# ChangwuLiu/InGVIO

Hardware: AMD Instinct MI355X
Metric: ekf_updates_per_sec (higher is better)
Workload: dtype f64; 1 GPU; BASELINE configs[1]: synthetic stereo MSCKF, 150 feats x 11 clones, state dim N=249 (update at N), 512 independent filters per GPU; step = propagate(k=10)+clone+MSCKF update+marginalise; filters_per_gpu=512, feats=150, clones=11, state_dim=249, imu_steps=10, parallelism=independent filters, 1 rank(s), no data-path collective

## Files before the change

### ingvio_amd/csrc/capi.hip

```cpp
#include "../../include/ingvio_hip.h"
#include "dev_common.h"
#include "launch_ekf.h"
#include "launch_msckf.h"
#include "launch_factored.h"
#include "launch_tri.h"
#include "launch_tracks.h"
#include "launch_lm.h"
#include "launch_delayed.h"
#include "launch_qr.h"
#include "launch_chol.h"
#include "launch_gnss.h"
#include "launch_lmbatch.h"
#include "launch_nominal.h"
#include "launch_tail.h"

#include <stdio.h>
#include <stdlib.h>
#include <string.h>
#include <unistd.h>
#include <string>
#include <atomic>
#include <cmath>
#include <condition_variable>
#include <functional>
#include <mutex>
#include <thread>
#include <utility>
#include <vector>

#define KMAX 64
#ifndef UPLOAD_KERNEL_MAX
#define UPLOAD_KERNEL_MAX (256u << 10)
#endif
#define IMU_SLAB_NB 4
#define CHI2_CAP 1024

namespace {

enum ProfId { PF_RESTORE, PF_PROPAGATE, PF_AUGMENT, PF_GATE, PF_FOLD, PF_MERGE, PF_EKF_CORE, PF_DOWNDATE, PF_MARG,
              PF_GATE2, PF_GRAM, PF_INFO, PF_APPLY, PF_ROWGATE, PF_LM_BUILD, PF_LM_GEMM, PF_LM_CHOL, PF_POSTCOLS, PF_COUNT };
const char* kProfNames[PF_COUNT] = { "restore", "k_propagate", "k_augment", "k_msckf_gate", "k_msckf_fold",
                                     "k_msckf_merge", "k_ekf_core", "k_downdate", "k_marginalize",
                                     "gate", "gram", "solve", "apply", "k_rows_gate",
                                     "k_lm_build", "k_lm_gemm", "k_lm_chol", "k_post_cols" };
struct ProfRec { int id; hipEvent_t a, b; };

}

struct ingvio_ctx {
    ingvio_ctx_desc d;
    int ldp, mld, nc_cap, G, rstride, hstride, cstride, ystride;
    int cls;
    hipStream_t st;
    bool own_stream;
    std::string err;
    double *Pbase, *Psnap;
    size_t pp = 0;
    int *d_cur, *d_n, *d_n_snap;
    std::vector<int> h_n, h_cur, h_n_snap;
    bool has_snap;
    int prof_only = -1;
    bool strip_ok = false;
    std::vector<int> h_nclones;
    struct { double *e = nullptr, *o = nullptr, *r = nullptr, *f = nullptr; int cap = 0; } se;
    bool phase_restore = false;
    unsigned long long mut_seq = 0, strip_seq = 0;
    double *d_Phi, *d_G, *d_dt, *d_R, *d_blk;
    double* d_prm = nullptr;
    int *d_gnss, *d_idx;
    int* d_zero_idx = nullptr;
    char* d_result_slab = nullptr;
    char* h_result = nullptr;
    size_t result_bytes = 0, ro_gam = 0, ro_used = 0, ro_m = 0, ro_st = 0, ro_tok = 0, ro_tpf = 0;
    char* d_frame_slab[2] = { nullptr, nullptr };
    int *d_clone_idx, *d_nclones, *d_nfeat, *d_anchor, *d_dof;
    double *d_clone_R, *d_clone_p, *d_pf, *d_uv, *d_chi2;
    unsigned long long* d_mask;
    double *d_gamma, *d_Rpart, *d_H, *d_res, *d_noise, *d_noise1, *d_Y, *d_Yc, *d_dx, *d_rec, *d_hnew;
    int method;
    int *d_accept, *d_used, *d_chunk_used, *d_colmap, *d_m, *d_nc, *d_status, *d_pcbase;
    double *d_big_sg, *d_big_wk;
    double* d_Asum = nullptr;
    int* d_used_sum = nullptr;
    struct { std::vector<double> chi2; bool chi2_ok = false; double var = 0.0; int b0 = -1, nb = 0; bool noise_ok = false; } upc;
    int apply_flipped = 0;
    bool fork_recorded = false;
    unsigned long long* d_tri_mask = nullptr;
    char* d_imu = nullptr;
    double* d_Tflat = nullptr;

    int* d_tri_ok;
    struct QrCache { int m = 0, n = 0, ldh = 0, chol = 0; double *dA = nullptr, *db = nullptr, *ws = nullptr, *dT = nullptr; hipGraphExec_t exec = nullptr; } qr;
    int qr_method = 0;
    double* d_noiseB = nullptr;
    struct GnssStage {
        double *H = nullptr, *res = nullptr, *noise = nullptr, *gamma = nullptr, *chi2 = nullptr;
        int *m = nullptr, *nc = nullptr, *colmap = nullptr, *keep = nullptr;
        double *feph = nullptr, *fobs = nullptr, *frcv = nullptr, *front = nullptr;
        int ncw = 0, m_cap = 0, n_vars_hi = 0, chi2_len = 0, gate_rows = 0, strong = 0;
        double thr1 = 0.0;
        std::vector<int> hi;
        bool staged = false;
        bool in_frame = false, fused_last = false;
        bool folded_last = false;
        bool results = false;
        int nc_max = 0;
        double *W = nullptr, *Yf = nullptr, *dxf = nullptr;
        int *mf = nullptr, *ncf = nullptr;
        bool nominal = false, nom_pending = false, own_status = false;
        bool frame_nom = false;
        int nom_b0 = 0, nom_nb = 0;
        int* stf = nullptr;
    } gn;
    struct DenseWs {
        double *Hd = nullptr, *X = nullptr, *Y = nullptr, *Tb = nullptr, *U = nullptr, *noise = nullptr, *noiseB = nullptr;
        int *m = nullptr, *cidx = nullptr, *rowmap = nullptr;
        int m_cap = 0, n_ld = 0, n32 = 0, ldx = 0;
        size_t hstride = 0, xstride = 0, tstride = 0, ustride = 0;
    } dw;
    struct LmStage {
        double *pose = nullptr, *pf = nullptr, *uv = nullptr, *gamma = nullptr, *dx = nullptr;
        int *idx = nullptr, *n_lm = nullptr, *lm_idx = nullptr, *anchor_idx = nullptr, *tracked = nullptr, *accept = nullptr;
        LmOpts op;
        int l_hi = 0, in_frame = 0;
        bool alloc = false, staged = false;
        int* slot = nullptr;
        bool nominal = false, nom_pending = false;
        int nom_b0 = 0, nom_nb = 0;
        std::vector<int> hi;
    } lm;
    char* d_multi = nullptr;
    struct DelayedWs { char *in = nullptr, *wk = nullptr, *out = nullptr, *h_out = nullptr; size_t in_cap = 0, wk_cap = 0, out_cap = 0; } dl;
    size_t multi_cap = 0;
    int st_stereo, st_enable_gnss, st_fmax_used;
    std::vector<double> st_prm;
    MsckfOpts st_op;
    std::vector<int> st_gnss;
    std::vector<int> st_marg;
    std::vector<int> st_cidx_hi;
    bool staged;
    double* d_xchg = nullptr;
    bool phase_pending = false;
    struct InputSet {
        double *Phi = nullptr, *G = nullptr, *dt = nullptr, *R = nullptr, *clone_R = nullptr, *clone_p = nullptr, *pf = nullptr, *uv = nullptr,
               *chi2 = nullptr, *noise = nullptr, *prm = nullptr;
        int *gnss = nullptr, *idx = nullptr, *clone_idx = nullptr, *nclones = nullptr, *nfeat = nullptr, *anchor = nullptr, *dof = nullptr;
        unsigned long long* mask = nullptr;
    } alt;
    bool alt_ready = false;
    hipStream_t st2 = nullptr;
    hipEvent_t ev_fork = nullptr, ev_join = nullptr, ev_ref = nullptr;
    hipEvent_t ev_fetch = nullptr;
    int fetch_b0 = 0, fetch_nb = 0;
    hipStream_t st_copy = nullptr;
    hipEvent_t ev_copy = nullptr, ev_free[2] = { nullptr, nullptr };
    bool copy_pending = false, free_valid[2] = { false, false };
    int set_id = 0;
    struct PinSlab { char* p = nullptr; size_t cap = 0; hipEvent_t ev = nullptr; bool busy = false; };
    PinSlab pin[4];
    int pin_next = 0;
    struct PartStream { hipStream_t st = nullptr; hipEvent_t ev_gate = nullptr, ev_apply = nullptr, ev_done = nullptr; };
    PartStream part[4];
    int parts_alloc = 0;
    int parts_req = -1;
    bool split_pending = false;
    hipEvent_t tok_last = nullptr;
    hipEvent_t ev_split_fork = nullptr;
    hipStream_t run_st = nullptr;
    hipEvent_t tok_wait = nullptr, tok_rec = nullptr;
    struct Tracks { double *uv = nullptr, *pf = nullptr; unsigned long long* mask = nullptr; int t_max = 0; char* stage[2] = { nullptr, nullptr }; size_t stage_cap = 0; } trk;
    struct Nominal {
        int vmax = 0, ir = 0, dr = 0;
        int* ih = nullptr; double* dv = nullptr;
        int* ih_snap = nullptr; double* dv_snap = nullptr;
        double* dx = nullptr;
        std::vector<int> h_ih, h_ih_snap;
        bool has_snap = false;
        bool pending = false;
        bool frame = false;
        hipEvent_t ev = nullptr; bool ev_valid = false;
    } nom;
    struct TailWs { char *in = nullptr, *ws = nullptr, *h_out = nullptr; size_t in_cap = 0, ws_cap = 0, out_cap = 0; } tl;
    bool prof;
    std::vector<ProfRec> recs;
    double prof_ms[PF_COUNT];
    int prof_calls[PF_COUNT];
};

namespace {

#define HIPCHK(ctx, expr)                                                                       \
    do {                                                                                        \
        hipError_t e__ = (expr);                                                                \
        if (e__ != hipSuccess) {                                                                \
            (ctx)->err = std::string(#expr) + ": " + hipGetErrorString(e__);                    \
            return INGVIO_E_HIP;                                                                \
        }                                                                                       \
    } while (0)

template <class T>
int dalloc(ingvio_ctx* c, T** p, size_t count)
{
    HIPCHK(c, hipMalloc((void**)p, sizeof(T) * (count ? count : 1)));
    HIPCHK(c, hipMemsetAsync(*p, 0, sizeof(T) * (count ? count : 1), c->st));
    return 0;
}

CovView view(ingvio_ctx* c)
{
    CovView v;
    v.Pbase = c->Pbase; v.cur = c->d_cur; v.n = c->d_n; v.ldp = c->ldp; v.B = c->d.batch; v.pstride = c->pp;
    ++c->mut_seq;
    return v;
}

FrameView fview(ingvio_ctx* c)
{
    FrameView f;
    f.clone_idx = c->d_clone_idx; f.clone_R = c->d_clone_R; f.clone_p = c->d_clone_p;
    f.n_clones = c->d_nclones; f.n_feat = c->d_nfeat; f.pf = c->d_pf; f.anchor = c->d_anchor;
    f.obs_mask = c->d_mask; f.uv = c->d_uv; f.dof = c->d_dof; f.cmax = c->d.c_max; f.fmax = c->d.f_max;
    return f;
}

struct ProfScope {
    ingvio_ctx* c; int id; hipEvent_t a, b; bool on;
    ProfScope(ingvio_ctx* c_, int id_) : c(c_), id(id_), on(c_->prof && (c_->prof_only < 0 || c_->prof_only == id_))
    {
        if (on) { hipEventCreate(&a); hipEventCreate(&b); hipEventRecord(a, c->run_st); }
    }
    ~ProfScope()
    {
        if (on) { hipEventRecord(b, c->run_st); c->recs.push_back({ id, a, b }); }
    }
};

int check_range(ingvio_ctx* c, int b0, int nb)
// ... 359 lines not shown
           pad64(8 * n * fm * cm * 4) + pad64(8 * n * fm) + 1024;
}

int validate_frames(ingvio_ctx* c, int b0, int nb, const ingvio_msckf_frame* fr, int grow, int* fmax_used)
{
    const int cm = c->d.c_max, fm = c->d.f_max;
    int fmx = 0;
    for (int i = 0; i < nb; ++i) {
        const ingvio_msckf_frame& f = fr[i];
        if (f.n_clones < 0 || f.n_clones > cm || f.n_feat < 0 || f.n_feat > fm) return INGVIO_E_CAPACITY;
        if (f.n_clones > 0 && (!f.clone_idx || !f.clone_R || !f.clone_p)) return INGVIO_E_ARG;
        if (f.n_feat > 0 && (!f.obs_mask || !f.uv)) return INGVIO_E_ARG;
        if (f.n_feat > fmx) fmx = f.n_feat;
        const int n_live = grow >= 0 ? c->h_n[b0 + i] + grow : c->d.n_max;
        const int n_lim = n_live < c->d.n_max ? n_live : c->d.n_max;
        for (int s = 0; s < f.n_clones; ++s) {
            if (f.clone_idx[s] < 0) return INGVIO_E_ARG;
            if (f.clone_idx[s] + 6 > n_lim) return f.clone_idx[s] + 6 > c->d.n_max ? INGVIO_E_ARG : INGVIO_E_NOT_IN_STATE;
        }
        if (f.anchor)
            for (int j = 0; j < f.n_feat; ++j) if (f.anchor[j] < 0 || f.anchor[j] >= f.n_clones) return INGVIO_E_ARG;
    }
    if (fmax_used) *fmax_used = fmx;
    return 0;
}

int pack_frames(ingvio_ctx* c, Uploader& up, int b0, int nb, const ingvio_msckf_frame* fr, int* fmax_used)
{
    const int cm = c->d.c_max, fm = c->d.f_max;
    int fmx = 0;
    for (int i = 0; i < nb; ++i) if (fr[i].n_feat > fmx) fmx = fr[i].n_feat;
    const bool whole = b0 == 0 && nb == c->d.batch;
    up.off = (up.off + 63) & ~(size_t)63;
    const size_t slab0 = up.off;
    int* cidx = up.take<int>((size_t)nb * cm); int* ncl = up.take<int>(nb); int* nft = up.take<int>(nb);
    int* anc = up.take<int>((size_t)nb * fm); int* dof = up.take<int>((size_t)nb * fm);
    double* cR = up.take<double>((size_t)nb * cm * 9); double* cp = up.take<double>((size_t)nb * cm * 3);
    double* pf = up.take<double>((size_t)nb * fm * 3);
    unsigned long long* mk = up.take<unsigned long long>((size_t)nb * fm);
    double* uv = up.take<double>((size_t)nb * fm * cm * 4);
    parallel_for(nb, [=](int i) {
        const ingvio_msckf_frame& f = fr[i];
        const int C = f.n_clones, F = f.n_feat;
        ncl[i] = C; nft[i] = F;
        memcpy(cidx + (size_t)i * cm, f.clone_idx, sizeof(int) * (size_t)C);
        memcpy(cR + (size_t)i * cm * 9, f.clone_R, 72 * (size_t)C);
        memcpy(cp + (size_t)i * cm * 3, f.clone_p, 24 * (size_t)C);
        if (f.pf) memcpy(pf + (size_t)i * fm * 3, f.pf, 24 * (size_t)F); else memset(pf + (size_t)i * fm * 3, 0, 24 * (size_t)F);
        if (f.anchor) memcpy(anc + (size_t)i * fm, f.anchor, sizeof(int) * (size_t)F); else memset(anc + (size_t)i * fm, 0, sizeof(int) * (size_t)F);
        if (f.dof) memcpy(dof + (size_t)i * fm, f.dof, sizeof(int) * (size_t)F); else memset(dof + (size_t)i * fm, 0, sizeof(int) * (size_t)F);
        const unsigned long long cmask = C >= 64 ? ~0ULL : ((1ULL << C) - 1ULL);
        unsigned long long* mki = mk + (size_t)i * fm;
        for (int j = 0; j < F; ++j) mki[j] = f.obs_mask[j] & cmask;
        for (int j = F; j < fm; ++j) mki[j] = 0ULL;
        double* uvi = uv + (size_t)i * fm * cm * 4;
        if (C == cm) memcpy(uvi, f.uv, 32 * (size_t)F * C);
        else for (int j = 0; j < F; ++j) memcpy(uvi + (size_t)j * cm * 4, f.uv + (size_t)j * C * 4, 32 * (size_t)C);
    });
    for (int i = 0; i < nb; ++i) c->h_nclones[b0 + i] = fr[i].n_clones;
    if (whole) {
        const size_t used = (size_t)(reinterpret_cast<char*>(uv) - (up.slab->p + slab0)) + 8 * ((size_t)(nb - 1) * fm + (size_t)fr[nb - 1].n_feat) * cm * 4;
        up.copy(reinterpret_cast<char*>(c->d_clone_idx), up.slab->p + slab0, std::max(used, (size_t)64));
        *fmax_used = fmx;
        return 0;
    }
    up.copy(c->d_clone_idx + (size_t)b0 * cm, cidx, (size_t)nb * cm);
    up.copy(c->d_nclones + b0, ncl, nb);
    up.copy(c->d_nfeat + b0, nft, nb);
    up.copy(c->d_anchor + (size_t)b0 * fm, anc, (size_t)nb * fm);
    up.copy(c->d_dof + (size_t)b0 * fm, dof, (size_t)nb * fm);
    up.copy(c->d_clone_R + (size_t)b0 * cm * 9, cR, (size_t)nb * cm * 9);
    up.copy(c->d_clone_p + (size_t)b0 * cm * 3, cp, (size_t)nb * cm * 3);
    up.copy(c->d_pf + (size_t)b0 * fm * 3, pf, (size_t)nb * fm * 3);
    up.copy(c->d_uv + (size_t)b0 * fm * cm * 4, uv, (size_t)nb * fm * cm * 4);
    up.copy(c->d_mask + (size_t)b0 * fm, mk, (size_t)nb * fm);
    *fmax_used = fmx;
    return 0;
}

int stage_frames(ingvio_ctx* c, int b0, int nb, const ingvio_msckf_frame* fr, int* fmax_used, int grow = 0)
{
    int rc = validate_frames(c, b0, nb, fr, grow, nullptr);
    if (rc) return rc;
    if (wait_inputs(c)) return INGVIO_E_HIP;
    Uploader up{ c };
    rc = up.begin(frames_bytes(c, nb));
    if (rc) return rc;
    pack_frames(c, up, b0, nb, fr, fmax_used);
    return up.end();
}

void fill_opts(const ingvio_ctx* c, const ingvio_msckf_opts* o, MsckfOpts* op)
{
    memcpy(op->R_lr, o->R_cl2cr, 72);
    memcpy(op->t_lr, o->t_cl2cr, 24);
    op->var = o->noise * o->noise;
    op->max_accept = o->max_accept;
    op->selected_variant = o->selected_variant;
    op->chi2 = c->d_chi2;
    op->chi2_len = o->chi2_len;
}

int make_opts(ingvio_ctx* c, const ingvio_msckf_opts* o, MsckfOpts* op)
{
    if (!o || !o->chi2_table || o->chi2_len < 2 || o->chi2_len > CHI2_CAP) return INGVIO_E_ARG;
    fill_opts(c, o, op);
    if (wait_inputs(c)) return INGVIO_E_HIP;
    auto& u = c->upc;
    if (u.chi2_ok && (int)u.chi2.size() >= o->chi2_len && !memcmp(u.chi2.data(), o->chi2_table, 8 * (size_t)o->chi2_len)) return 0;
    const UpItem item = { c->d_chi2, o->chi2_table, 8 * (size_t)o->chi2_len };
    if (stage_small(c, &item, 1)) return INGVIO_E_HIP;
    u.chi2.assign(o->chi2_table, o->chi2_table + o->chi2_len); u.chi2_ok = true;
    return 0;
}

#define GNSS_NCW 32

void gnss_front_launch(ingvio_ctx* c, int b0, int nb, bool nominal, hipStream_t st);
static int gnss_in_frame_launch(ingvio_ctx* c, int b0, int nb, FactoredLaunch& L)
{
    auto& g = c->gn;
    const size_t mld = c->mld, hs = mld * GNSS_NCW, ws = (size_t)c->ldp * 16;
    L.gcolmap = g.colmap + (size_t)b0 * GNSS_NCW; L.gnc = g.nc + b0; L.gcstride = GNSS_NCW;
    L.gW = g.W + (size_t)b0 * ws; L.gWstride = ws;
    if (g.frame_nom) {
        L.stage = 10; launch_factored(L, c->run_st);
        launch_nominal_update(nom_table(c), c->d_dx, c->ldp, nullptr, b0, nb, c->run_st);
        gnss_front_launch(c, b0, nb, true, c->run_st);
    }
    { ProfScope p(c, PF_POSTCOLS); L.stage = 4; launch_factored(L, c->run_st); }
    EkfLaunch E;
    memset(&E, 0, sizeof E);
    E.cv = L.cv; E.b0 = b0; E.nb = nb; E.H = c->d_H + (size_t)b0 * hs; E.res = c->d_res + (size_t)b0 * mld;
    E.colmap = c->d_colmap + (size_t)b0 * GNSS_NCW; E.m = g.mf + b0; E.nc = g.ncf + b0;
    E.noise = c->d_noiseB + (size_t)b0 * mld; E.r_kind = INGVIO_R_DIAG; E.mld = c->mld; E.hstride = (int)hs; E.cstride = GNSS_NCW;
    E.nstride = c->mld; E.Y = g.Yf + (size_t)b0 * ws; E.ystride = (int)ws; E.dx = g.dxf;
    E.status = g.own_status ? g.stf : c->d_status; E.m_cap = g.m_cap; E.nc_cap = GNSS_NCW;
    E.W = L.gW; E.wstride = ws; E.ypad = 16; E.marg_idx = L.marg_idx; E.marg_size = L.marg_size;
    if (g.strong) { E.chi2 = g.chi2; E.chi2_len = g.chi2_len; E.gate_max_rows = 14; }
    RowsGateIn in{ g.H + (size_t)b0 * hs, g.res + (size_t)b0 * mld, g.noise + (size_t)b0 * mld, g.m + b0, g.colmap + (size_t)b0 * GNSS_NCW,
                   g.nc + b0, (int)hs, GNSS_NCW };
    {
        ProfScope p(c, PF_ROWGATE);
        if (launch_rows_gate(E, in, g.thr1, g.gamma + (size_t)b0 * mld, g.keep + (size_t)b0 * mld, c->run_st)) return INGVIO_E_CAPACITY;
    }
    { ProfScope p(c, PF_EKF_CORE); launch_ekf_core(E, c->run_st); }
    L.gY = E.Y; L.gYstride = ws; L.gm = g.mf + b0;
    g.fused_last = true; g.folded_last = true;
    g.results = true;
    return 0;
}

int run_msckf_factored(ingvio_ctx* c, int b0, int nb, const MsckfOpts& op, int stereo, int fmax_used,
                       const int* marg_idx = nullptr, int marg_size = 0, int phase = 0, bool gnss_fuse = false)
{
    FactoredLaunch L;
    memset(&L, 0, sizeof L);
    L.stereo = stereo; L.cv = view(c); L.fv = fview(c); L.op = op; L.b0 = b0; L.nb = nb;
    L.fmax_used = fmax_used > 0 ? fmax_used : 1;
    L.ncol_cap = 6 * c->d.c_max;
    for (int i = 0; i < nb; ++i) if (c->h_nclones[b0 + i] > L.c_used) L.c_used = c->h_nclones[b0 + i];
    L.gamma = c->d_gamma; L.accept = c->d_accept; L.used = c->d_used; L.rec = c->d_rec;
    L.Apart = c->d_Rpart + (size_t)b0 * c->G * c->rstride; L.chunk_used = c->d_chunk_used + (size_t)b0 * c->G;
    L.G = c->G; L.rstride = c->rstride; L.noise = c->d_noise + b0;
    L.Tflat = c->d_Tflat; L.tfstride = (size_t)c->ldp * 100; L.flat_nb = std::min(c->d.batch, APPLY_FLAT_NB);
    L.Asum = c->d_Asum ? c->d_Asum + (size_t)b0 * c->rstride : nullptr; L.used_sum = c->d_used_sum ? c->d_used_sum + b0 : nullptr;
#ifdef INGVIO_ALT_KERNELS
    static const bool few_off = [] { const char* e = getenv("INGVIO_FEW"); return e && !strcmp(e, "off"); }();
    if (few_off) { L.Tflat = nullptr; L.Asum = nullptr; }
#endif
    L.T = c->d_Y + (size_t)b0 * c->ystride; L.Pc = c->d_Yc + (size_t)b0 * c->ystride; L.ystride = c->ystride;
    L.dx = c->d_dx; L.m_out = c->d_m + b0; L.nc_out = c->d_nc + b0; L.status = c->d_status;
    L.big_sg = c->d_big_sg ? c->d_big_sg + (size_t)b0 * bigwin_sg_doubles(c->G) : nullptr;
    L.big_wk = c->d_big_wk ? c->d_big_wk + (size_t)b0 * bigwin_wk_doubles() : nullptr;
    const bool big = c->d.c_max > 16;
    L.mstride = c->ystride; L.n_cap = c->d.n_max;
    L.marg_idx = marg_idx; L.marg_size = marg_size; L.pc_base = c->d_pcbase + b0;
    c->apply_flipped = 0;
    L.flip_cnt = c->d_pcbase + c->d.batch + b0; L.did_flip = no_apply_flip() ? nullptr : &c->apply_flipped;
    bool forked = false;
    if (big && phase == 0 && c->st2) {
        if (!c->fork_recorded) HIPCHK(c, hipEventRecord(c->ev_fork, c->run_st));
        c->fork_recorded = false;
        forked = true;
    }
    if (phase != 2) {
        if (c->tok_wait) HIPCHK(c, hipStreamWaitEvent(c->run_st, c->tok_wait, 0));
        {
            const bool pon = c->prof && (c->prof_only < 0 || c->prof_only == PF_GATE2);
            int used = 0;
            if (pon) { hipEventCreate(&L.prof_a); hipEventCreate(&L.prof_b); L.prof_used = &used; }
            L.stage = 0;
            const int grc = launch_factored(L, c->run_st);
            if (pon) {
                if (used) c->recs.push_back({ PF_GATE2, L.prof_a, L.prof_b });
                else { hipEventDestroy(L.prof_a); hipEventDestroy(L.prof_b); }
                L.prof_a = nullptr; L.prof_b = nullptr; L.prof_used = nullptr;
            }
            if (grc) return INGVIO_E_UNSUPPORTED;
        }
        { ProfScope p(c, PF_GRAM); L.stage = 1; launch_factored(L, c->run_st); }
        if (c->tok_rec) HIPCHK(c, hipEventRecord(c->tok_rec, c->run_st));
    }
    if (forked) {
        HIPCHK(c, hipStreamWaitEvent(c->st2, c->ev_fork, 0));
        L.stage = 6; launch_factored(L, c->st2);
        HIPCHK(c, hipEventRecord(c->ev_ref, c->st2));
        L.stage = 7; launch_factored(L, c->st2);
        HIPCHK(c, hipEventRecord(c->ev_join, c->st2));
    }
    if (phase == 1) return last_launch(c);
    if (forked) {
        ProfScope p(c, PF_INFO);
        HIPCHK(c, hipStreamWaitEvent(c->run_st, c->ev_ref, 0));
        L.stage = 8; launch_factored(L, c->run_st);
        HIPCHK(c, hipStreamWaitEvent(c->run_st, c->ev_join, 0));
        L.stage = 9; launch_factored(L, c->run_st);
    } else {
        if (big) { ProfScope p(c, PF_INFO); L.stage = 5; launch_factored(L, c->run_st); }
        { ProfScope p(c, PF_INFO); L.stage = 2; launch_factored(L, c->run_st); }
    }
    if (gnss_fuse) { if (int rc = gnss_in_frame_launch(c, b0, nb, L)) return rc; }
    if (phase == 2 && c->tok_wait) HIPCHK(c, hipStreamWaitEvent(c->run_st, c->tok_wait, 0));
    { ProfScope p(c, PF_APPLY); L.stage = 3; launch_factored(L, c->run_st); }
    if (phase == 2 && c->tok_rec) HIPCHK(c, hipEventRecord(c->tok_rec, c->run_st));
    return last_launch(c);
}

int run_msckf(ingvio_ctx* c, int b0, int nb, const MsckfOpts& op, int stereo, int fmax_used)
{
    if (c->method == 1) return run_msckf_factored(c, b0, nb, op, stereo, fmax_used);
    MsckfLaunch L;
    memset(&L, 0, sizeof L);
    L.stereo = stereo; L.cv = view(c); L.fv = fview(c); L.op = op; L.b0 = b0; L.nb = nb;
    L.fmax_used = fmax_used > 0 ? fmax_used : 1;
    L.gamma = c->d_gamma; L.accept = c->d_accept; L.used = c->d_used;
    L.Rpart = c->d_Rpart + (size_t)b0 * c->G * c->rstride; L.chunk_used = c->d_chunk_used + (size_t)b0 * c->G;
    L.G = c->G; L.rstride = c->rstride;
    L.Hout = c->d_H + (size_t)b0 * c->hstride; L.res_out = c->d_res + (size_t)b0 * c->mld;
    L.colmap = c->d_colmap + (size_t)b0 * c->cstride; L.m_out = c->d_m + b0; L.nc_out = c->d_nc + b0;
    L.mld = c->mld; L.hstride = c->hstride; L.cstride = c->cstride;
    { ProfScope p(c, PF_GATE); L.stage = 0; if (launch_msckf(L, c->st)) return INGVIO_E_UNSUPPORTED; }
    { ProfScope p(c, PF_FOLD); L.stage = 1; launch_msckf(L, c->st); }
    { ProfScope p(c, PF_MERGE); L.stage = 2; launch_msckf(L, c->st); }
    EkfLaunch E;
    memset(&E, 0, sizeof E);
    E.cv = view(c); E.b0 = b0; E.nb = nb; E.H = L.Hout; E.res = L.res_out; E.colmap = L.colmap; E.m = L.m_out; E.nc = L.nc_out;
    E.noise = c->d_noise + b0; E.r_kind = 0; E.mld = c->mld; E.hstride = c->hstride; E.cstride = c->cstride; E.nstride = 1;
    E.Y = c->d_Y + (size_t)b0 * c->ystride; E.ystride = c->ystride; E.dx = c->d_dx; E.status = c->d_status;
    E.m_cap = 6 * c->d.c_max; E.nc_cap = 6 * c->d.c_max;
    { ProfScope p(c, PF_EKF_CORE); launch_ekf_core(E, c->st); }
    { ProfScope p(c, PF_DOWNDATE); launch_downdate(E, c->d.n_max, c->st); }
    return last_launch(c);
}

int fill_noise_scalar(ingvio_ctx* c, int b0, int nb, double var)
{
    auto& u = c->upc;
    if (u.noise_ok && u.b0 == b0 && u.nb == nb && u.var == var) return 0;
    std::vector<double> v(nb, var);
    const UpItem item = { c->d_noise + b0, v.data(), 8 * (size_t)nb };
    if (stage_small(c, &item, 1)) return INGVIO_E_HIP;
    u.noise_ok = true; u.b0 = b0; u.nb = nb; u.var = var;
    return 0;
}

template <class Step>
int stage_imu_params(ingvio_ctx* c, int b0, int nb, const Step* steps, const double sigma[4], double scb, double srw, double* blk, int* count)
{
    const bool all = !c->staged;
    const int lo = all ? 0 : b0, hi = all ? c->d.batch : b0 + nb;
    for (int b = lo; b < hi; ++b) {
        double* h = &c->st_prm[(size_t)b * 8];
        h[0] = sigma[0]; h[1] = sigma[1]; h[2] = sigma[2]; h[3] = sigma[3]; h[4] = scb; h[5] = srw;
        h[6] = (double)steps[b >= b0 && b < b0 + nb ? b - b0 : 0].k; h[7] = 0.0;
        memcpy(blk + (size_t)(b - lo) * 8, h, 64);
    }
    *count = hi - lo;
    return lo;
}

struct FrameStage {
    ingvio_ctx* c; int b0, nb; const ingvio_msckf_opts* opts; const double* sigma; int enable_gnss; double scb, srw; bool async;
    Uploader upl{ c };
    int refuse(bool inputs, bool tracks) const
    {
        if (phase_busy(c)) return INGVIO_E_ARG;
        if (c && c->nom.pending) { c->err = "a frame staged from the device nominal state has not run yet"; return INGVIO_E_ARG; }
        if (check_range(c, b0, nb) || !inputs || !opts || !sigma) return INGVIO_E_ARG;
        if (tracks && !c->trk.t_max) { c->err = "ingvio_frame_stage_tracks without ingvio_tracks_create"; return INGVIO_E_ARG; }
        if (async && (b0 != 0 || nb != c->d.batch)) return INGVIO_E_ARG;
        if (!opts->chi2_table || opts->chi2_len < 2 || opts->chi2_len > CHI2_CAP) return INGVIO_E_ARG;
        return 0;
    }
    int begin(size_t bytes)
    {
        if (async) if (int rc = prepare_async_set(c)) return rc;
        return upl.begin(bytes + pad64(8 * CHI2_CAP) + pad64(8 * (size_t)nb) + pad64(64 * (size_t)c->d.batch) + 1024);
    }
    int fail(int code)
    {
        hipStreamSynchronize(c->st);
        if (c->st_copy) hipStreamSynchronize(c->st_copy);
        c->staged = false; c->copy_pending = false;
        return code;
    }
    template <class Step>
    int commit(const Step* steps)
    {
        bool same = c->staged && enable_gnss == c->st_enable_gnss;
        for (int i = 0; i < nb; ++i)
            for (int g = 0; g < 5; ++g) {
                int& old = c->st_gnss[(size_t)(b0 + i) * 5 + g];
                if (old != steps[i].gnss_idx[g]) { same = false; old = steps[i].gnss_idx[g]; }
            }
// ... 2817 lines not shown
    return INGVIO_OK;
}

static bool lm_in_frame(const ingvio_ctx* c) { return c->lm.staged && c->lm.in_frame; }
static bool gnss_in_frame(const ingvio_ctx* c) { return c->gn.staged && c->gn.in_frame && c->gn.m_cap > 0; }
static bool gnss_folds(const ingvio_ctx* c)
{
    if (!gnss_in_frame(c) || c->d.c_max > 16 || c->gn.m_cap > 16 || c->gn.nc_max > 16) return false;
    for (int b = 0; b < c->d.batch; ++b) if (c->st_marg[b] < 0 || c->gn.hi[b] > c->st_marg[b]) return false;
    return true;
}

static bool strips_valid(const ingvio_ctx* c, int restore_prior) { return restore_prior && c->strip_ok && c->mut_seq == c->strip_seq; }

static void launch_restore_propagate(ingvio_ctx* c, int restore_prior, bool strips, int b0, int nb, hipStream_t st)
{
    const bool from_snap = strips && propagate_can_restore(c->d.n_max) && !no_snap_propagate();
    if (restore_prior && !from_snap) {
        ProfScope p(c, PF_RESTORE);
        if (strips) launch_restore_strips(view(c), b0, nb, c->d.n_max, c->Psnap, c->d_n_snap, c->st_enable_gnss ? c->d_gnss : nullptr, st);
        else launch_restore(view(c), b0, nb, c->d.n_max, c->Psnap, c->d_n_snap, st);
    }
    ProfScope p(c, PF_PROPAGATE);
    const ImuLaunch im = imu_launch(c, b0, nb);
    launch_propagate(view(c), b0, nb, c->d.n_max, c->d_Phi + (size_t)b0 * KMAX * 225, c->d_G + (size_t)b0 * KMAX * 180, c->d_dt + (size_t)b0 * KMAX,
                     im.k, KMAX, im.prm, c->st_enable_gnss ? c->d_gnss + (size_t)b0 * 5 : nullptr, im.sigma, c->st_enable_gnss, im.scb, im.srw, st,
                     c->d_R + (size_t)b0 * 9, c->d_status, from_snap ? c->Psnap : nullptr, c->d_n_snap);
}

static void mirror_restore_clone(ingvio_ctx* c, int restore_prior)
{
    if (restore_prior) { c->h_n = c->h_n_snap; std::fill(c->h_cur.begin(), c->h_cur.end(), 0); }
    for (int b = 0; b < c->d.batch; ++b) c->h_n[b] += 6;
}
static bool mirror_marg(ingvio_ctx* c)
{
    bool all = true;
    for (int b = 0; b < c->d.batch; ++b) { if (c->st_marg[b] >= 0) { c->h_n[b] -= 6; c->h_cur[b] ^= 1; } else all = false; }
    return all;
}

static void consume_in_frame(bool& staged, bool in_frame, bool replay) { if (staged && in_frame && !replay) staged = false; }
static void strips_after_step(ingvio_ctx* c, bool valid) { c->strip_ok = valid; c->strip_seq = c->mut_seq; }

static int frame_run_split(ingvio_ctx* c, int restore_prior, int P, bool gnss_fuse)
{
    const int B = c->d.batch;
    if (parts_prepare(c, P)) return INGVIO_E_HIP;
    if (c->split_pending && c->copy_pending) ENTER(c);
    if (wait_inputs(c)) return INGVIO_E_HIP;
    if (!c->split_pending) {
        HIPCHK(c, hipEventRecord(c->ev_split_fork, c->st));
        for (int p = 0; p < P; ++p) HIPCHK(c, hipStreamWaitEvent(c->part[p].st, c->ev_split_fork, 0));
        c->tok_last = nullptr;
    }
    const bool strips = strips_valid(c, restore_prior);
    mirror_restore_clone(c, restore_prior);
    int rc = 0;
    auto range = [&](int p, int& b0, int& nb) {
        b0 = (int)((long long)B * p / P) & ~7;
        const int b1 = p + 1 == P ? B : ((int)((long long)B * (p + 1) / P) & ~7);
        nb = b1 - b0;
    };
    for (int p = 0; p < P && !rc; ++p) {
        int b0, nb; range(p, b0, nb);
        if (nb <= 0) continue;
        auto& q = c->part[p];
        c->run_st = q.st;
        launch_restore_propagate(c, restore_prior, strips, b0, nb, q.st);
        c->tok_wait = c->tok_last; c->tok_rec = q.ev_gate;
        rc = run_msckf_factored(c, b0, nb, c->st_op, c->st_stereo, c->st_fmax_used, c->d_idx + b0, 6, 1, gnss_fuse);
        c->tok_last = rc ? nullptr : q.ev_gate;
    }
    for (int p = 0; p < P && !rc; ++p) {
        int b0, nb; range(p, b0, nb);
        if (nb <= 0) continue;
        auto& q = c->part[p];
        c->run_st = q.st;
        c->tok_wait = c->tok_last; c->tok_rec = q.ev_apply;
        rc = run_msckf_factored(c, b0, nb, c->st_op, c->st_stereo, c->st_fmax_used, c->d_idx + b0, 6, 2, gnss_fuse);
        c->tok_last = rc ? nullptr : q.ev_apply;
        if (!rc && !c->apply_flipped) {
            ProfScope pr(c, PF_MARG);
            launch_post_marg(view(c), b0, nb, c->d_idx + b0, 6, q.st);
        }
    }
    for (int p = 0; p < P; ++p) hipEventRecord(c->part[p].ev_done, c->part[p].st);
    c->tok_wait = nullptr; c->tok_rec = nullptr;
    c->run_st = c->st;
    c->split_pending = true;
    if (rc) { c->tok_last = nullptr; ENTER(c); return rc; }
    const bool all_marg = mirror_marg(c);
    strips_after_step(c, all_marg && restore_prior);
    consume_in_frame(c->gn.staged, c->gn.in_frame, restore_prior != 0);
    return INGVIO_OK;
}

static int frame_run_front(ingvio_ctx* c, int restore_prior)
{
    const int B = c->d.batch;
    ENTER(c);
    if (wait_inputs(c)) return INGVIO_E_HIP;
    launch_restore_propagate(c, restore_prior, strips_valid(c, restore_prior), 0, B, c->st);
    mirror_restore_clone(c, restore_prior);
    strips_after_step(c, false);
    const int rc = run_msckf_factored(c, 0, B, c->st_op, c->st_stereo, c->st_fmax_used, nullptr, 0, 1);
    if (rc == 0) { c->phase_pending = true; c->phase_restore = restore_prior != 0; }
    return rc;
}

static int frame_run_back(ingvio_ctx* c)
{
    c->phase_pending = false;
    const int B = c->d.batch;
    const bool with_lm = lm_in_frame(c), replay = c->phase_restore;
    int rc = run_msckf_factored(c, 0, B, c->st_op, c->st_stereo, c->st_fmax_used, with_lm ? nullptr : c->d_idx, with_lm ? 0 : 6, 2);
    if (rc) return rc;
    if (with_lm) { rc = landmark_update_launch(c, 0, B); if (rc) return rc; }
    {
        ProfScope p(c, PF_MARG);
        if (!with_lm) { if (!c->apply_flipped) launch_post_marg(view(c), 0, B, c->d_idx, 6, c->st); }
        else launch_marginalize(view(c), 0, B, c->d.n_max, c->d_idx, 6, c->st);
    }
    mirror_marg(c);
    consume_in_frame(c->lm.staged, c->lm.in_frame, replay);
    strips_after_step(c, false);
    if (gnss_in_frame(c)) {
        rc = gnss_run_separate(c, 0, B, true);
        if (rc) return rc;
        consume_in_frame(c->gn.staged, c->gn.in_frame, replay);
    }
    return release_input_set(c);
}

static int frame_run_whole(ingvio_ctx* c, int restore_prior)
{
    const int B = c->d.batch;
    ENTER(c);
    if (wait_inputs(c)) return INGVIO_E_HIP;
    launch_restore_propagate(c, restore_prior, strips_valid(c, restore_prior), 0, B, c->st);
    mirror_restore_clone(c, restore_prior);
    const bool with_lm = lm_in_frame(c);
    const bool fuse = c->method == 1 && !with_lm;
    const bool lm_oop = with_lm && c->method == 1;
    const bool gnss_here = gnss_in_frame(c), gnss_fuse = fuse && gnss_folds(c);
    const bool gnss_nomf = c->gn.staged && c->gn.frame_nom;
    if (gnss_nomf) {
        auto& g = c->gn;
        HIPCHK(c, hipMemsetAsync(g.dxf, 0, 8 * (size_t)B * c->ldp, c->st));
        HIPCHK(c, hipMemsetAsync(g.stf, 0, sizeof(int) * (size_t)B, c->st));
        HIPCHK(c, hipMemsetAsync(g.mf, 0, sizeof(int) * (size_t)B, c->st));
        g.own_status = true; g.results = true; g.fused_last = true; g.folded_last = false;
    }
    int rc = fuse     ? run_msckf_factored(c, 0, B, c->st_op, c->st_stereo, c->st_fmax_used, c->d_idx, 6, 0, gnss_fuse)
             : lm_oop ? run_msckf_factored(c, 0, B, c->st_op, c->st_stereo, c->st_fmax_used, c->d_zero_idx, 0)
                      : run_msckf(c, 0, B, c->st_op, c->st_stereo, c->st_fmax_used);
    if (rc) return rc;
    if (lm_oop) {
        if (!c->apply_flipped) launch_post_marg(view(c), 0, B, c->d_zero_idx, 0, c->st);
        for (int b = 0; b < B; ++b) c->h_cur[b] ^= 1;
    }
    const bool lm_nom = with_lm && c->lm.nominal;
    if (lm_nom) landmark_gather_launch(c, c->d_dx, 0, B);
    bool lm_fused = false;
    if (with_lm) { rc = landmark_update_launch(c, 0, B, c->d_idx, 6, &lm_fused); if (rc) return rc; }
    if (!(fuse && c->apply_flipped)) {
        ProfScope p(c, PF_MARG);
        if (fuse || lm_fused) launch_post_marg(view(c), 0, B, c->d_idx, 6, c->st);
        else launch_marginalize(view(c), 0, B, c->d.n_max, c->d_idx, 6, c->st);
    }
    consume_in_frame(c->lm.staged, c->lm.in_frame, restore_prior != 0);
    const bool all_marg = mirror_marg(c);
    if (c->nom.pending) {
        if (gnss_nomf && gnss_fuse) launch_nominal_update_post(nom_table(c), c->gn.dxf, c->ldp, c->d_idx, 0, B, c->st);
        else launch_nominal_update(nom_table(c), lm_nom ? c->lm.dx : c->d_dx, c->ldp, c->d_idx, 0, B, c->st);
        if (int rc2 = last_launch(c)) return rc2;
        for (int b = 0; b < B; ++b) nom_mirror_marg(c, b, c->st_marg[b]);
        c->nom.pending = false;
        if (nom_mark(c)) return INGVIO_E_HIP;
    }
    strips_after_step(c, fuse && all_marg && restore_prior);
    if (gnss_here && !gnss_fuse) {
        if (gnss_nomf) {
            for (int b = 0; b < B; ++b) { int& hi = c->gn.hi[b]; if (c->st_marg[b] >= 0 && hi > c->st_marg[b]) hi -= 6; }
            gnss_front_launch(c, 0, B, true, c->st);
        }
        rc = gnss_run_separate(c, 0, B, true);
        if (rc) return rc;
        if (gnss_nomf) {
            launch_nominal_update(nom_table(c), c->gn.dxf, c->ldp, nullptr, 0, B, c->st);
            if (int rc2 = last_launch(c)) return rc2;
            if (nom_mark(c)) return INGVIO_E_HIP;
        }
    }
    consume_in_frame(c->gn.staged, c->gn.in_frame, restore_prior != 0);
    if (!c->gn.staged) c->gn.frame_nom = false;
    return release_input_set(c);
}

static int frame_run_impl(ingvio_ctx* c, int restore_prior, int phase)
{
    if (!c || !c->staged) return INGVIO_E_ARG;
    if (c->nom.frame) {
        if (!c->nom.pending) { c->err = "the frame staged from the device nominal state has already run"; return INGVIO_E_ARG; }
        if (phase) { c->err = "the split step does not take a frame staged from the device nominal state"; return INGVIO_E_UNSUPPORTED; }
        if (restore_prior) { c->err = "restore_prior with a frame staged from the device nominal state (restore with ingvio_cov_restore before the stage)"; return INGVIO_E_ARG; }
        if ((c->gn.staged && c->gn.in_frame && !c->gn.frame_nom) || (lm_in_frame(c) && !c->lm.nominal) || c->parts_req > 1) {
            c->err = "the device nominal state takes no in-frame GNSS / host-fed landmark stage and frame_parts = 1 only"; return INGVIO_E_UNSUPPORTED;
        }
    } else if (lm_in_frame(c) && c->lm.nominal) {
        c->err = "an in-frame landmark stage from the device nominal state needs a frame staged from it"; return INGVIO_E_ARG;
    } else if (c->gn.staged && c->gn.frame_nom) {
        c->err = "a GNSS epoch staged for a frame from the device nominal state needs that frame"; return INGVIO_E_ARG;
    }
    if (phase && c->method != 1) return INGVIO_E_UNSUPPORTED;
    if (phase != 2 && phase_busy(c)) return INGVIO_E_ARG;
    if (phase == 2 && !c->phase_pending) { c->err = "ingvio_frame_run_phase(.., 2) without a preceding phase 1"; return INGVIO_E_ARG; }
    if (phase != 0 && c->st_op.max_accept > 0) { c->err = "max_accept is not supported by the split (feature-sharded) frame step"; return INGVIO_E_ARG; }
    if (phase == 2) return frame_run_back(c);
    const int B = c->d.batch;
    if (restore_prior && !c->has_snap) return INGVIO_E_ARG;
    if (c->method == 0 && c->d.c_max > 16) return INGVIO_E_UNSUPPORTED;
    {
        const std::vector<int>& n0 = restore_prior ? c->h_n_snap : c->h_n;
        for (int b = 0; b < B; ++b) {
            if (n0[b] < 21) return INGVIO_E_ARG;
            if (n0[b] + 6 > c->d.n_max) return INGVIO_E_CAPACITY;
            if (c->st_cidx_hi[b] + 6 > n0[b] + 6) return INGVIO_E_NOT_IN_STATE;
            if (c->st_marg[b] >= 0 && c->st_marg[b] + 6 > n0[b] + 6) return INGVIO_E_NOT_IN_STATE;
        }
        if (lm_in_frame(c)) { if (int rc = landmark_in_state(c, 0, B, n0, 6)) return rc; }
    }
    if (phase == 1) return frame_run_front(c, restore_prior);
    const int P = std::min(c->parts_req > 0 ? c->parts_req : 1, 4);
    const bool gnss_fuse = gnss_folds(c);
    if (P > 1 && c->method == 1 && !lm_in_frame(c) && c->d.c_max <= 16 && (!gnss_in_frame(c) || gnss_fuse) && B >= 16 * P)
        return frame_run_split(c, restore_prior, P, gnss_fuse);
    return frame_run_whole(c, restore_prior);
}

int ingvio_frame_run(ingvio_ctx* c, int restore_prior) { return frame_run_impl(c, restore_prior, 0); }
int ingvio_set_frame_parts(ingvio_ctx* c, int parts)
{
    if (!c || parts < -1 || parts > 4) return INGVIO_E_ARG;
    ENTER(c);
    c->parts_req = parts == 0 ? 1 : parts;
    return INGVIO_OK;
}
int ingvio_frame_run_phase(ingvio_ctx* c, int restore_prior, int phase)
{
    if (phase < 0 || phase > 2) return INGVIO_E_ARG;
    return frame_run_impl(c, restore_prior, phase);
}

int ingvio_info_set(ingvio_ctx* c, int b, const double* A, int ncol, int n_accepted)
{
    ENTER(c);
    if (check_range(c, b, 1) || !A || ncol < 6 || (size_t)ncol * (ncol + 1) > (size_t)c->rstride || n_accepted < 0) return INGVIO_E_ARG;
    std::vector<int> used(c->G, 0);
    used[0] = n_accepted;
    int rc = up(c, c->d_Rpart + (size_t)b * c->G * c->rstride, A, 8 * (size_t)ncol * (ncol + 1));
    rc |= up(c, c->d_chunk_used + (size_t)b * c->G, used.data(), sizeof(int) * (size_t)c->G);
    if (rc) return INGVIO_E_HIP;
    HIPCHK(c, hipStreamSynchronize(c->st));
    return INGVIO_OK;
}

namespace {
__global__ __launch_bounds__(256) void k_info_reduce(const double* __restrict__ Apart, const int* __restrict__ chunk_used, int G, int rstride,
                                                     int cnt, double* __restrict__ out)
{
    const int e = blockIdx.x * 256 + threadIdx.x;
    if (e > cnt) return;
    double s = 0.0;
    if (e < cnt) { for (int g = 0; g < G; ++g) if (chunk_used[g]) s += Apart[(size_t)g * rstride + e]; }
    else { for (int g = 0; g < G; ++g) s += (double)chunk_used[g]; }
    out[e] = s;
}
__global__ __launch_bounds__(256) void k_info_commit(const double* __restrict__ in, int cnt, double* __restrict__ Apart0, int* __restrict__ chunk_used, int G)
{
    const int e = blockIdx.x * 256 + threadIdx.x;
    if (e < cnt) Apart0[e] = in[e];
    if (e < G) chunk_used[e] = e == 0 ? (int)llrint(in[cnt]) : 0;
}
}

int ingvio_info_reduce(ingvio_ctx* c, int b, double** dev_ptr, int* count, int* ncol_out)
{
    ENTER(c);
    if (check_range(c, b, 1) || !dev_ptr || !count || c->method != 1) return INGVIO_E_ARG;
    int C = 0;
    if (down_sync(c, &C, c->d_nclones + b, sizeof(int))) return INGVIO_E_HIP;
    const int ncol = 6 * C, cnt = ncol * (ncol + 1);
    if (cnt <= 0 || cnt > c->rstride) return INGVIO_E_ARG;
    if (!c->d_xchg && dalloc(c, &c->d_xchg, (size_t)c->d.batch * (c->rstride + 8))) return INGVIO_E_HIP;
    double* out = c->d_xchg + (size_t)b * (c->rstride + 8);
    hipLaunchKernelGGL(k_info_reduce, dim3((cnt + 256) / 256), dim3(256), 0, c->st, c->d_Rpart + (size_t)b * c->G * c->rstride,
                       c->d_chunk_used + (size_t)b * c->G, c->G, c->rstride, cnt, out);
    HIPCHK(c, hipStreamSynchronize(c->st));
    *dev_ptr = out; *count = cnt + 1;
    if (ncol_out) *ncol_out = ncol;
    return last_launch(c);
}

int ingvio_info_commit(ingvio_ctx* c, int b)
{
    ENTER(c);
    if (check_range(c, b, 1) || !c->d_xchg || c->method != 1) return INGVIO_E_ARG;
    int C = 0;
    if (down_sync(c, &C, c->d_nclones + b, sizeof(int))) return INGVIO_E_HIP;
    const int ncol = 6 * C, cnt = ncol * (ncol + 1);
    if (cnt <= 0 || cnt > c->rstride) return INGVIO_E_ARG;
    hipLaunchKernelGGL(k_info_commit, dim3((std::max(cnt, c->G) + 255) / 256), dim3(256), 0, c->st, c->d_xchg + (size_t)b * (c->rstride + 8), cnt,
                       c->d_Rpart + (size_t)b * c->G * c->rstride, c->d_chunk_used + (size_t)b * c->G, c->G);
    return last_launch(c);
}

int ingvio_frame_fetch_begin(ingvio_ctx* c, int b0, int nb)
{
    ENTER(c);
    if (check_range(c, b0, nb)) return INGVIO_E_ARG;
    const int fm = c->d.f_max;
    if (!c->ev_fetch) HIPCHK(c, hipEventCreateWithFlags(&c->ev_fetch, hipEventDisableTiming));
    HIPCHK(c, hipMemcpyAsync(c->h_result + 8 * (size_t)b0 * c->ldp, c->d_dx + (size_t)b0 * c->ldp, 8 * (size_t)nb * c->ldp, hipMemcpyDeviceToHost, c->st));
    HIPCHK(c, hipMemcpyAsync(c->h_result + c->ro_used + sizeof(int) * (size_t)b0 * fm, c->d_used + (size_t)b0 * fm, sizeof(int) * (size_t)nb * fm, hipMemcpyDeviceToHost, c->st));
    HIPCHK(c, hipMemcpyAsync(c->h_result + c->ro_m + sizeof(int) * (size_t)b0, c->d_m + b0, sizeof(int) * (size_t)nb, hipMemcpyDeviceToHost, c->st));
    HIPCHK(c, hipEventRecord(c->ev_fetch, c->st));
    c->fetch_b0 = b0; c->fetch_nb = nb;
    return last_launch(c);
}

int ingvio_frame_fetch_end(ingvio_ctx* c, double* dx_out, int* accepted, int* rows_out)
{
    if (!c || c->fetch_nb <= 0) return INGVIO_E_ARG;
    const int fm = c->d.f_max, b0 = c->fetch_b0, nb = c->fetch_nb;
    HIPCHK(c, hipEventSynchronize(c->ev_fetch));
    c->fetch_nb = 0;
    if (dx_out) memcpy(dx_out, c->h_result + 8 * (size_t)b0 * c->ldp, 8 * (size_t)nb * c->ldp);
    if (accepted) memcpy(accepted, c->h_result + c->ro_used + sizeof(int) * (size_t)b0 * fm, sizeof(int) * (size_t)nb * fm);
    if (rows_out) memcpy(rows_out, c->h_result + c->ro_m + sizeof(int) * (size_t)b0, sizeof(int) * (size_t)nb);
    return INGVIO_OK;
}

int ingvio_frame_fetch(ingvio_ctx* c, int b0, int nb, double* dx_out, int* accepted, int* rows_out)
{
    int rc = ingvio_frame_fetch_begin(c, b0, nb);
    if (rc) return rc;
    rc = ingvio_frame_fetch_end(c, dx_out, accepted, rows_out);
    if (rc) return rc;
    HIPCHK(c, hipStreamSynchronize(c->st));
    return last_launch(c);
}

int ingvio_set_msckf_method(ingvio_ctx* c, int method)
{
    ENTER(c);
    if (!c || method < 0 || method > 1) return INGVIO_E_ARG;
    c->method = method;
    return INGVIO_OK;
}

int ingvio_debug_msckf_info(ingvio_ctx* c, int b, double* A_out, int* ncol_out)
{
    ENTER(c);
    if (check_range(c, b, 1) || !A_out || !ncol_out) return INGVIO_E_ARG;
    int C = 0;
    if (down_sync(c, &C, c->d_nclones + b, sizeof(int))) return INGVIO_E_HIP;
    const int ncol = 6 * C;
    *ncol_out = ncol;
    const size_t w = (size_t)ncol + 1;
    for (size_t e = 0; e < (size_t)ncol * w; ++e) A_out[e] = 0.0;
    if (c->method == 1) {
        std::vector<int> used(c->G);
        if (down_sync(c, used.data(), c->d_chunk_used + (size_t)b * c->G, sizeof(int) * (size_t)c->G)) return INGVIO_E_HIP;
        std::vector<double> part((size_t)ncol * w);
        for (int g = 0; g < c->G; ++g) {
            if (!used[g]) continue;
            if (down_sync(c, part.data(), c->d_Rpart + ((size_t)b * c->G + g) * c->rstride, 8 * part.size())) return INGVIO_E_HIP;
            for (size_t e = 0; e < part.size(); ++e) A_out[e] += part[e];
        }
        return INGVIO_OK;
    }
    int m = 0;
    if (down_sync(c, &m, c->d_m + b, sizeof(int))) return INGVIO_E_HIP;
    if (m == 0) return INGVIO_OK;
    std::vector<double> R((size_t)c->mld * ncol), z(c->mld);
    if (down_sync(c, R.data(), c->d_H + (size_t)b * c->hstride, 8 * R.size()) || down_sync(c, z.data(), c->d_res + (size_t)b * c->mld, 8 * (size_t)ncol))
        return INGVIO_E_HIP;
    for (int i = 0; i < ncol; ++i) {
        for (int j = 0; j < ncol; ++j) {
            double a = 0.0;
            for (int k = 0; k <= (i < j ? i : j); ++k) a += R[k + (size_t)i * c->mld] * R[k + (size_t)j * c->mld];
            A_out[i * w + j] = a;
        }
        double bb = 0.0;
        for (int k = 0; k <= i; ++k) bb += R[k + (size_t)i * c->mld] * z[k];
        A_out[i * w + ncol] = bb;
    }
    return INGVIO_OK;
}

int ingvio_debug_info_solution(ingvio_ctx* c, int b, double* out, int count)
{
    ENTER(c);
    if (check_range(c, b, 1) || !out || count < 1 || count > c->ystride) return INGVIO_E_ARG;
    if (down_sync(c, out, c->d_Y + (size_t)b * c->ystride, 8 * (size_t)count)) return INGVIO_E_HIP;
    return INGVIO_OK;
}

static int debug_quiesce(ingvio_ctx* c)
{
    HIPCHK(c, hipStreamSynchronize(c->st));
    if (c->st_copy) HIPCHK(c, hipStreamSynchronize(c->st_copy));
    return 0;
}
static int debug_down(ingvio_ctx* c, void* dst, const void* src, size_t bytes)
{
    if (dst && bytes) HIPCHK(c, hipMemcpy(dst, src, bytes, hipMemcpyDeviceToHost));
    return 0;
}

int ingvio_debug_tracks_read(ingvio_ctx* c, int b, unsigned long long* mask, double* uv, double* pf)
{
    ENTER(c);
    if (check_range(c, b, 1)) return INGVIO_E_ARG;
    if (!c->trk.t_max) { c->err = "ingvio_debug_tracks_read without ingvio_tracks_create"; return INGVIO_E_ARG; }
    if (debug_quiesce(c)) return INGVIO_E_HIP;
    const size_t T = c->trk.t_max, C = c->d.c_max;
    if (debug_down(c, mask, c->trk.mask + (size_t)b * T, 8 * T) || debug_down(c, uv, c->trk.uv + (size_t)b * T * C * 4, 8 * T * C * 4) ||
        debug_down(c, pf, c->trk.pf + (size_t)b * T * 3, 8 * T * 3)) return INGVIO_E_HIP;
    return INGVIO_OK;
}

int ingvio_debug_staged_frame(ingvio_ctx* c, int b, int* n_clones, int* n_feat, int* clone_idx, double* clone_R, double* clone_p, int* anchor, int* dof,
                              unsigned long long* obs_mask, double* pf, double* uv)
{
    ENTER(c);
    if (check_range(c, b, 1)) return INGVIO_E_ARG;
    if (debug_quiesce(c)) return INGVIO_E_HIP;
    const size_t cm = c->d.c_max, fm = c->d.f_max, B = b;
    if (debug_down(c, n_clones, c->d_nclones + B, 4) || debug_down(c, n_feat, c->d_nfeat + B, 4) ||
        debug_down(c, clone_idx, c->d_clone_idx + B * cm, 4 * cm) || debug_down(c, clone_R, c->d_clone_R + B * cm * 9, 8 * cm * 9) ||
        debug_down(c, clone_p, c->d_clone_p + B * cm * 3, 8 * cm * 3) || debug_down(c, anchor, c->d_anchor + B * fm, 4 * fm) ||
        debug_down(c, dof, c->d_dof + B * fm, 4 * fm) || debug_down(c, obs_mask, c->d_mask + B * fm, 8 * fm) ||
        debug_down(c, pf, c->d_pf + B * fm * 3, 8 * fm * 3) || debug_down(c, uv, c->d_uv + B * fm * cm * 4, 8 * fm * cm * 4)) return INGVIO_E_HIP;
    return INGVIO_OK;
}

int ingvio_debug_read(ingvio_ctx* c, long long* out, int n)
{
    ENTER(c);
    if (!c || !out || n < 1 || n > 64) return INGVIO_E_ARG;
    HIPCHK(c, hipStreamSynchronize(c->st));
    long long a[64], bq[64], cq[64], sq[64];
    if (dbg_read_factored(a, 64) || dbg_read_cov(bq, 64) || dbg_read_bigwin(cq, 64) || dbg_read_solve(sq, 64)) return INGVIO_E_HIP;
    long long hq[64];
    if (dbg_read_chol(hq, 64)) return INGVIO_E_HIP;
    long long lq[64], mq[64];
    if (dbg_read_lmbatch(lq, 64) || dbg_read_lmchol(mq, 64)) return INGVIO_E_HIP;
    if (const char* e = getenv("INGVIO_DBG_TU")) {
        const long long* src = e[0] == 'b' ? cq : (e[0] == 'c' ? hq : (e[0] == 's' ? sq : (e[0] == 'l' ? lq : (e[0] == 'm' ? mq : a))));
        for (int i = 0; i < n; ++i) out[i] = src[i];
        return INGVIO_OK;
    }
    for (int i = 0; i < n; ++i)
        out[i] = i >= 56 ? hq[i - 56] : (i >= 48 ? cq[i] : ((i >= 24 && i < 32) ? sq[i - 24] : ((i < 16 || i >= 32) ? a[i] : bq[i])));
    return INGVIO_OK;
}

int ingvio_profile_select(ingvio_ctx* c, const char* kernel_name)
{
    ENTER(c);
    if (!c) return INGVIO_E_ARG;
    c->prof_only = -1;
    if (!kernel_name || !*kernel_name) return INGVIO_OK;
    for (int i = 0; i < PF_COUNT; ++i) if (!strcmp(kernel_name, kProfNames[i])) { c->prof_only = i; return INGVIO_OK; }
    return INGVIO_E_ARG;
}

int ingvio_profile_enable(ingvio_ctx* c, int enable)
{
    ENTER(c);
    if (!c) return INGVIO_E_ARG;
    c->prof = enable != 0;
    return INGVIO_OK;
}

static void prof_collect(ingvio_ctx* c)
{
    hipStreamSynchronize(c->st);
    for (auto& r : c->recs) {
        float ms = 0.f;
        if (hipEventElapsedTime(&ms, r.a, r.b) == hipSuccess) { c->prof_ms[r.id] += ms; c->prof_calls[r.id] += 1; }
        hipEventDestroy(r.a); hipEventDestroy(r.b);
    }
    c->recs.clear();
}

int ingvio_profile_reset(ingvio_ctx* c)
{
    ENTER(c);
    if (!c) return INGVIO_E_ARG;
    prof_collect(c);
    memset(c->prof_ms, 0, sizeof c->prof_ms); memset(c->prof_calls, 0, sizeof c->prof_calls);
    return INGVIO_OK;
}

int ingvio_profile_get(ingvio_ctx* c, const char** names, double* ms, int* calls, int cap)
{
    ENTER(c);
    if (!c || !names || !ms || !calls) return INGVIO_E_ARG;
    prof_collect(c);
    int k = 0;
    for (int i = 0; i < PF_COUNT && k < cap; ++i) { names[k] = kProfNames[i]; ms[k] = c->prof_ms[i]; calls[k] = c->prof_calls[i]; ++k; }
    return k;
}

}
// ... 1 lines not shown
```

### ingvio_amd/csrc/feat_build.h

```cpp
#pragma once
#include "dev_common.h"

template <int CMAX, bool STEREO>
struct FeatCfg {
    static constexpr int RPO = STEREO ? 4 : 2;
    static constexpr int RR = RPO * CMAX;
    static constexpr int RRH = RR - 3;
    static constexpr int NCOLMAX = 6 * CMAX;
    static constexpr int NT = ((NCOLMAX + 1 + 63) / 64) * 64;
};

template <int CMAX, bool STEREO, bool LEAN>
struct FeatDenseOnly {
    using Cfg = FeatCfg<CMAX, STEREO>;
    double GX[CMAX][Cfg::RPO][3];
    double V[3][Cfg::RR];
    double tau[3];
};
template <int CMAX, bool STEREO>
struct FeatDenseOnly<CMAX, STEREO, true> {};

template <int CMAX, bool STEREO, bool LEAN = false>
struct FeatShared : FeatDenseOnly<CMAX, STEREO, LEAN> {
    using Cfg = FeatCfg<CMAX, STEREO>;
    static constexpr bool kLean = LEAN;
    double G[CMAX][Cfg::RPO][3];
    double res[CMAX][Cfg::RPO];
    int slot[CMAX];
    int gidx[LEAN ? CMAX : Cfg::NCOLMAX];
    int nobs;
};

template <bool STEREO>
__device__ __forceinline__ bool feat_obs(const double* R, const double* p, const double z[4], double pfx, double pfy,
                                         double pfz, const MsckfOpts& op, double (*Gm)[3], double* rs)
{
    constexpr int RPO = STEREO ? 4 : 2;
    const double dx = pfx - p[0], dy = pfy - p[1], dz = pfz - p[2];
    double q[3], Rt[9];
#pragma unroll
    for (int i = 0; i < 3; ++i) {
        q[i] = R[i] * dx + R[3 + i] * dy + R[6 + i] * dz;
        Rt[3 * i] = R[i]; Rt[3 * i + 1] = R[3 + i]; Rt[3 * i + 2] = R[6 + i];
    }
    const double iz = q[2] == 0.0 ? __builtin_copysign(__builtin_inf(), q[2]) : fast_rcp(q[2]);
    const double hp02 = -q[0] * (iz * iz), hp12 = -q[1] * (iz * iz);
#pragma unroll
    for (int m = 0; m < 3; ++m) {
        Gm[0][m] = iz * Rt[m] + hp02 * Rt[6 + m];
        Gm[1][m] = iz * Rt[3 + m] + hp12 * Rt[6 + m];
    }
    rs[0] = z[0] - q[0] * iz;
    rs[1] = z[1] - q[1] * iz;
    bool nan = (iz != iz) || (hp02 != hp02) || (hp12 != hp12);
#pragma unroll
    for (int i = 0; i < 9; ++i) nan |= (R[i] != R[i]);
    nan |= (pfx != pfx) || (pfy != pfy) || (pfz != pfz);
    if (STEREO) {
        double qr[3], M[9];
#pragma unroll
        for (int i = 0; i < 3; ++i)
            qr[i] = op.R_lr[3 * i] * q[0] + op.R_lr[3 * i + 1] * q[1] + op.R_lr[3 * i + 2] * q[2] + op.t_lr[i];
#pragma unroll
        for (int i = 0; i < 3; ++i)
#pragma unroll
            for (int m = 0; m < 3; ++m)
                M[3 * i + m] = op.R_lr[3 * i] * Rt[m] + op.R_lr[3 * i + 1] * Rt[3 + m] + op.R_lr[3 * i + 2] * Rt[6 + m];
        const double izr = qr[2] == 0.0 ? __builtin_copysign(__builtin_inf(), qr[2]) : fast_rcp(qr[2]);
        const double h02 = -qr[0] * (izr * izr), h12 = -qr[1] * (izr * izr);
#pragma unroll
        for (int m = 0; m < 3; ++m) {
            Gm[RPO - 2][m] = izr * M[m] + h02 * M[6 + m];
            Gm[RPO - 1][m] = izr * M[3 + m] + h12 * M[6 + m];
        }
        rs[RPO - 2] = z[2] - qr[0] * izr;
        rs[RPO - 1] = z[3] - qr[1] * izr;
    }
    return !nan;
}

template <int CMAX, bool STEREO, bool LEAN = false>
__device__ __forceinline__ int feat_phase1(const FrameView& fv, const MsckfOpts& op, int b, int j, int C,
                                           FeatShared<CMAX, STEREO, LEAN>& sh)
{
    using Cfg = FeatCfg<CMAX, STEREO>;
    constexpr int RPO = Cfg::RPO;
    const int tid = threadIdx.x;
    const double* pf = fv.pf + ((size_t)b * fv.fmax + j) * 3;
    const double pfx = pf[0], pfy = pf[1], pfz = pf[2];
    const unsigned long long mask = fv.obs_mask[(size_t)b * fv.fmax + j];
    if (tid < WAVE) {
        const int s = tid;
        bool valid = false;
        double Gm[RPO][3], rs[RPO];
        if (s < C && ((mask >> s) & 1ULL)) {
            const double* R = fv.clone_R + ((size_t)b * fv.cmax + s) * 9;
            const double* p = fv.clone_p + ((size_t)b * fv.cmax + s) * 3;
            const double* z = fv.uv + (((size_t)b * fv.fmax + j) * fv.cmax + s) * 4;
            double zz[4] = { z[0], z[1], 0.0, 0.0 };
            if (STEREO) { zz[2] = z[2]; zz[3] = z[3]; }
            valid = feat_obs<STEREO>(R, p, zz, pfx, pfy, pfz, op, Gm, rs);
        }
        const unsigned long long vm = __ballot(valid);
        if (valid) {
            const int od = __popcll(vm & ((1ULL << s) - 1ULL));
            sh.slot[od] = s;
#pragma unroll
            for (int t = 0; t < RPO; ++t) {
#pragma unroll
                for (int m = 0; m < 3; ++m) sh.G[od][t][m] = Gm[t][m];
                if constexpr (!LEAN) {
                    sh.GX[od][t][0] = Gm[t][1] * pfz - Gm[t][2] * pfy;
                    sh.GX[od][t][1] = -Gm[t][0] * pfz + Gm[t][2] * pfx;
                    sh.GX[od][t][2] = Gm[t][0] * pfy - Gm[t][1] * pfx;
                }
                sh.res[od][t] = rs[t];
            }
        }
        if (tid == 0) sh.nobs = __popcll(vm);
    }
    __syncthreads();
    return RPO * sh.nobs;
}

template <int CMAX, bool STEREO>
__device__ __forceinline__ void feat_phase2(FeatShared<CMAX, STEREO>& sh, int rows)
{
    using Cfg = FeatCfg<CMAX, STEREO>;
    constexpr int RPO = Cfg::RPO, RR = Cfg::RR;
    const int tid = threadIdx.x;
    if (tid < WAVE) {
        constexpr int PER = (RR + WAVE - 1) / WAVE;
        double hf[3][PER];
#pragma unroll
        for (int u = 0; u < PER; ++u) {
            const int i = tid + u * WAVE;
#pragma unroll
            for (int m = 0; m < 3; ++m) hf[m][u] = (i < rows) ? sh.G[i / RPO][i % RPO][m] : 0.0;
        }
#pragma unroll
        for (int k = 0; k < 3; ++k) {
            double part = 0.0;
#pragma unroll
            for (int u = 0; u < PER; ++u) { const int i = tid + u * WAVE; if (i >= k) part += hf[k][u] * hf[k][u]; }
            const double nrm = sqrt(wave_sum(part));
            const double x0 = __shfl(hf[k][0], k, WAVE);
            double tau = 0.0, v0 = 1.0;
            if (nrm > 0.0) {
                const double alpha = x0 >= 0.0 ? -nrm : nrm;
                v0 = x0 - alpha;
                tau = -v0 / alpha;
            }
            double v[PER];
#pragma unroll
            for (int u = 0; u < PER; ++u) {
                const int i = tid + u * WAVE;
                v[u] = (nrm > 0.0) ? (i == k ? 1.0 : (i > k ? hf[k][u] / v0 : 0.0)) : 0.0;
                if (i < RR) sh.V[k][i] = v[u];
            }
#pragma unroll
            for (int c2 = k + 1; c2 < 3; ++c2) {
                double w = 0.0;
#pragma unroll
                for (int u = 0; u < PER; ++u) w += v[u] * hf[c2][u];
                w = wave_sum(w) * tau;
#pragma unroll
                for (int u = 0; u < PER; ++u) hf[c2][u] -= w * v[u];
            }
            if (tid == 0) sh.tau[k] = tau;
        }
    }
    __syncthreads();

}

template <int CMAX, bool STEREO, bool LEAN = false>
__device__ __forceinline__ void load_gidx(const FrameView& fv, int b, int C, FeatShared<CMAX, STEREO, LEAN>& sh)
{
    if constexpr (LEAN) {
        for (int c = threadIdx.x; c < C; c += blockDim.x) sh.gidx[c] = fv.clone_idx[(size_t)b * fv.cmax + c];
    } else {
        for (int c = threadIdx.x; c < 6 * C; c += blockDim.x)
            sh.gidx[c] = fv.clone_idx[(size_t)b * fv.cmax + c / 6] + c % 6;
    }
}
```

### ingvio_amd/csrc/gate5_kernel.h

```cpp
#pragma once
#include "gate_kernel.h"

#ifdef GATE5_RCP1
__device__ __forceinline__ double g5_rcp1(double x) { double r = __builtin_amdgcn_rcp(x); return fma(fma(-x, r, 1.0), r, r); }
#define G5RCP(x) g5_rcp1(x)
#else
#define G5RCP(x) fast_rcp(x)
#endif

template <int CMAX>
struct Gate5Shared {
    static constexpr int NF = 4;
    static constexpr int NR = CMAX - 1, NPMAX = 3 * NR, NTL = (NPMAX + 1 + 15) / 16, BR = 16 * NTL - 1, KPK = NPMAX * (NPMAX + 1) / 2;
    struct Feat {
        double vNinv[CMAX][9];
        double Rb[CMAX][9];
        double Q[9];
        double w[3 * CMAX];
        double rpsum;
        double thr;
    } f[NF];
    static constexpr int KPS = (KPK + 16 + 1) & ~1;
#ifndef GATE5_DB
#define GATE5_DB 1
#endif
    union alignas(16) {
        double kp[GATE5_DB ? 2 : 1][KPS];
        double pan[NF][16 * NTL][4];
        double fin[NF][16][18];
    };
    alignas(16) double lf[NF][20];
};

template <int CMAX>
__device__ __forceinline__ void gate5_body(CovView cv, FrameView fv, MsckfOpts op, int b0, int nb, int fmax_used, double* __restrict__ gamma_out,
                                           int* __restrict__ accept_out)
{
    using SH = Gate5Shared<CMAX>;
    constexpr int NF = SH::NF, NTL = SH::NTL, NLT = NTL * (NTL + 1) / 2, NPMAX = SH::NPMAX;
    static_assert(CMAX <= 16 && CMAX * (CMAX - 1) / 2 <= WAVE && NPMAX < 16 * NTL, "window class");
    __shared__ SH sh;
    const int ngrp = (fmax_used + NF - 1) / NF;
    const int wg = blockIdx.x, xcd = wg & 7, t = wg >> 3;
    const int bl = xcd + 8 * (t / ngrp), j0 = NF * (t % ngrp);
    if (bl >= nb) return;
    const int b = b0 + bl, lane = threadIdx.x & (WAVE - 1);
    const int F = fv.n_feat[b];
    if (j0 >= F) return;
    const int C = fv.n_clones[b], ld = cv.ldp;
    const double* P = cov_ptr(cv, b);
    dbg_stamp(5);
    const int g = lane >> 4, sl = lane & 15, gbase = lane & 48;
    const bool jok = j0 + g < F;
    const size_t oidx = (size_t)b * fv.fmax + (jok ? j0 + g : j0);
    const int a = fv.anchor[oidx];
    const double* pf = fv.pf + oidx * 3;
    const double px = pf[0], py = pf[1], pz = pf[2];
    const unsigned long long mask = jok ? fv.obs_mask[oidx] : 0ULL;
    const int cidx = sl < C ? fv.clone_idx[(size_t)b * fv.cmax + sl] : 0;
    const int npair = C * (C - 1) / 2;
    const bool pact = lane < npair;
    int pi = 0, pi2 = 0;
    {
        const int q = pact ? lane : 0;
        pi = (int)((sqrtf(8.0f * q + 1.0f) - 1.0f) * 0.5f);
        while ((pi + 1) * (pi + 2) / 2 <= q) ++pi;
        while (pi * (pi + 1) / 2 > q) --pi;
        pi2 = q - pi * (pi + 1) / 2;
    }
    const int pc = pi + 1, pc2 = pi2 + 1;
    const int gc = __shfl(cidx, pc, WAVE), gc2 = __shfl(cidx, pc2, WAVE);
    double Att[9], Atp[9], Apt[9], App[9];
    if (pact) {
#pragma unroll
        for (int m = 0; m < 3; ++m)
#pragma unroll
            for (int q = 0; q < 3; ++q) {
                Att[3 * m + q] = P[(gc + m) + (size_t)(gc2 + q) * ld];
                Atp[3 * m + q] = P[(gc + m) + (size_t)(gc2 + 3 + q) * ld];
                Apt[3 * m + q] = P[(gc + 3 + m) + (size_t)(gc2 + q) * ld];
                App[3 * m + q] = P[(gc + 3 + m) + (size_t)(gc2 + 3 + q) * ld];
            }
    }
    bool valid = false;
    double Gm[4][3], rs[4];
    if (sl < C && ((mask >> sl) & 1ULL)) {
        const double* R = fv.clone_R + ((size_t)b * fv.cmax + sl) * 9;
        const double* pp = fv.clone_p + ((size_t)b * fv.cmax + sl) * 3;
        const double* z = fv.uv + (oidx * fv.cmax + sl) * 4;
        const double zz[4] = { z[0], z[1], z[2], z[3] };
        valid = feat_obs<true>(R, pp, zz, px, py, pz, op, Gm, rs);
    }
    const unsigned long long vm = __ballot(valid);
    const unsigned gm = (unsigned)(vm >> gbase) & 0xFFFFu;
    const int bslot = gm ? __ffs(gm) - 1 : 0;
    const int od = __popc(gm & ((1u << sl) - 1u));
    const double plo = (valid && !(op.selected_variant && sl == a)) ? 1.0 : 0.0;
    const double plb = !(op.selected_variant && bslot == a) ? 1.0 : 0.0;
    const int gb = __shfl(cidx, gbase + bslot, WAVE);
    double u[3] = { 0.0, 0.0, 0.0 }, Ni[9], rr = 0.0;
#pragma unroll
    for (int i = 0; i < 9; ++i) Ni[i] = 0.0;
    if (valid) {
        double N[9], h[3];
#pragma unroll
        for (int m = 0; m < 3; ++m) {
#pragma unroll
            for (int m2 = m; m2 < 3; ++m2) {
                double sN = 0.0;
#pragma unroll
                for (int q = 0; q < 4; ++q) sN += Gm[q][m] * Gm[q][m2];
                N[3 * m + m2] = sN; N[3 * m2 + m] = sN;
            }
            double hh = 0.0;
#pragma unroll
            for (int q = 0; q < 4; ++q) hh += Gm[q][m] * rs[q];
            h[m] = hh;
        }
        inv3sym(N, Ni);
#pragma unroll
        for (int q = 0; q < 4; ++q) rr += rs[q] * rs[q];
#pragma unroll
        for (int m = 0; m < 3; ++m) {
            u[m] = Ni[3 * m] * h[0] + Ni[3 * m + 1] * h[1] + Ni[3 * m + 2] * h[2];
            rr -= h[m] * u[m];
        }
    }
#pragma unroll
    for (int off = 8; off > 0; off >>= 1) rr += __shfl_xor(rr, off, WAVE);
    double ub[3];
#pragma unroll
    for (int m = 0; m < 3; ++m) ub[m] = __shfl(u[m], gbase + bslot, WAVE);
    if (sl == 0) {
        sh.f[g].rpsum = rr;
        const int dof = fv.dof[oidx];
        sh.f[g].thr = (dof >= 1 && dof < op.chi2_len) ? op.chi2[dof] : -__builtin_inf();
    }
    if (valid) {
        typename SH::Feat& fg = sh.f[g];
#pragma unroll
        for (int i = 0; i < 9; ++i) fg.vNinv[sl][i] = op.var * Ni[i];
        if (od > 0) {
#pragma unroll
            for (int m = 0; m < 3; ++m) fg.w[3 * (od - 1) + m] = u[m] - ub[m];
        }
        double Rb[9];
        gate4_pairblock(P, ld, cidx, gb, plo, plb, px, py, pz, Rb);
        if (od == 0) {
#pragma unroll
            for (int i = 0; i < 9; ++i) fg.Q[i] = Rb[i] + op.var * Ni[i];
        } else {
#pragma unroll
            for (int i = 0; i < 9; ++i) fg.Rb[sl][i] = Rb[i];
        }
    }
    unsigned vmg[NF];
    int np_g[NF], bs_g[NF];
    bool fok_g[NF];
#pragma unroll
    for (int q = 0; q < NF; ++q) {
        vmg[q] = (unsigned)(vm >> (16 * q)) & 0xFFFFu;
        const int nobs = __popc(vmg[q]);
        fok_g[q] = nobs > 0;
        np_g[q] = nobs > 0 ? 3 * (nobs - 1) : 0;
        bs_g[q] = vmg[q] ? __ffs(vmg[q]) - 1 : 0;
    }
    wave_sync();
    dbg_stamp(7);
#if defined(GATE5_STOP_AFTER) && GATE5_STOP_AFTER == 1
    if (lane < NF && j0 + lane < F) { gamma_out[(size_t)b * fv.fmax + j0 + lane] = sh.f[lane].Q[0] + sh.f[lane].w[0] + sh.f[lane].rpsum; accept_out[(size_t)b * fv.fmax + j0 + lane] = 0; }
    return;
#endif
    bool need = false;
#pragma unroll
    for (int q = 0; q < NF; ++q) need |= ((vmg[q] >> pc) & 1u) && ((vmg[q] >> pc2) & 1u) && pc2 != bs_g[q];
    need = need && pact;
    const int kq = lane >> 4, l15 = lane & 15;
    const double mk0 = kq == 0 ? 1.0 : 0.0, mk1 = kq == 1 ? 1.0 : 0.0, mk2 = kq == 2 ? 1.0 : 0.0, mk3 = kq == 3 ? 1.0 : 0.0;
    double qx[NF], qy[NF], qz[NF];
    int aq[NF];
#pragma unroll
    for (int fq = 0; fq < NF; ++fq) {
        const size_t oq = (size_t)b * fv.fmax + (j0 + fq < F ? j0 + fq : j0);
        qx[fq] = fv.pf[oq * 3]; qy[fq] = fv.pf[oq * 3 + 1]; qz[fq] = fv.pf[oq * 3 + 2];
        aq[fq] = fv.anchor[oq];
    }
    auto pair_blocks = [&](int fq) {
        const unsigned vq = vmg[fq];
        if (need && ((vq >> pc) & 1u) && ((vq >> pc2) & 1u) && pc2 != bs_g[fq]) {
            const double pl = !(op.selected_variant && pc == aq[fq]) ? 1.0 : 0.0, pl2 = !(op.selected_variant && pc2 == aq[fq]) ? 1.0 : 0.0;
            double Su[9];
            gate5_fpf(Att, Atp, Apt, App, pl, pl2, qx[fq], qy[fq], qz[fq], Su);
            const typename SH::Feat& fg = sh.f[fq];
#pragma unroll
            for (int m = 0; m < 3; ++m)
#pragma unroll
                for (int k = 0; k < 3; ++k) Su[3 * m + k] += fg.Q[3 * m + k] - fg.Rb[pc][3 * m + k] - fg.Rb[pc2][3 * k + m];
            if (pc == pc2) {
#pragma unroll
                for (int k = 0; k < 9; ++k) Su[k] += fg.vNinv[pc][k];
            }
            const int i = __popc(vq & ((1u << pc) - 1u)) - 1, i2 = __popc(vq & ((1u << pc2) - 1u)) - 1;
            double* kp = sh.kp[GATE5_DB ? (fq & 1) : 0];
            int tri = (3 * i) * (3 * i + 1) / 2 + 3 * i2;
#pragma unroll
            for (int a2 = 0; a2 < 3; ++a2) {
#pragma unroll
                for (int c2 = 0; c2 < 3; ++c2)
                    if (i != i2 || c2 <= a2) kp[tri + c2] = Su[3 * a2 + c2];
                tri += 3 * i + a2 + 1;
            }
        }
    };
    double4_f T[NF][NLT];
    int fidx[NLT][4], wcol[NTL];
    bool fdiag[NLT][4];
#pragma unroll
    for (int ti = 0; ti < NTL; ++ti)
#pragma unroll
        for (int tj = 0; tj <= ti; ++tj)
#pragma unroll
            for (int r = 0; r < 4; ++r) {
                const int i = 16 * ti + kq + 4 * r, jc = 16 * tj + l15;
                const int hi = i > jc ? i : jc, lo = i > jc ? jc : i;
                const int e = hi * (hi + 1) / 2 + lo;
                fidx[ti * (ti + 1) / 2 + tj][r] = e < SH::KPK + 16 ? e : SH::KPK + 15;
                fdiag[ti * (ti + 1) / 2 + tj][r] = i == jc;
            }
#pragma unroll
    for (int tj = 0; tj < NTL; ++tj) wcol[tj] = 16 * tj + l15 < 3 * CMAX ? 16 * tj + l15 : 0;
    if (GATE5_DB) { pair_blocks(0); wave_sync(); }
#pragma unroll
    for (int fq = 0; fq < NF; ++fq) {
        if (GATE5_DB) { if (fq + 1 < NF) pair_blocks(fq + 1); }
        else { pair_blocks(fq); wave_sync(); }
        const int np = np_g[fq];
        const double* kp = sh.kp[GATE5_DB ? (fq & 1) : 0];
        const double* wq = sh.f[fq].w;
        bool jreal[NTL];
#pragma unroll
        for (int tj = 0; tj < NTL; ++tj) jreal[tj] = 16 * tj + l15 < np;
#ifndef GATE5_FILL_PIN1
#pragma unroll
        for (int t = 0; t < NLT; ++t)
#pragma unroll
            for (int r = 0; r < 4; ++r) T[fq][t][r] = kp[fidx[t][r]];
        double wvv[NTL];
#pragma unroll
        for (int tj = 0; tj < NTL; ++tj) wvv[tj] = wq[wcol[tj]];
#pragma unroll
        for (int ti = 0; ti < NTL; ++ti) {
#pragma unroll
            for (int tj = 0; tj <= ti; ++tj) {
                const int t = ti * (ti + 1) / 2 + tj;
                double b0 = T[fq][t][0], b1 = T[fq][t][1], b2 = T[fq][t][2], b3 = T[fq][t][3];
                PIN4(b0, b1, b2, b3);
                const double bvs[4] = { b0, b1, b2, b3 };
#pragma unroll
                for (int r = 0; r < 4; ++r) {
                    const bool ireal = 16 * ti + kq + 4 * r < np;
                    const double padv = (fdiag[t][r] && !ireal) ? 1.0 : 0.0;
                    double v = (ireal && jreal[tj]) ? bvs[r] : padv;
                    if (ti == NTL - 1 && r == 3) v = kq == 3 ? (jreal[tj] ? wvv[tj] : 0.0) : v;
                    T[fq][t][r] = v;
                }
            }
        }
#else
#pragma unroll
        for (int ti = 0; ti < NTL; ++ti) {
#pragma unroll
            for (int r = 0; r < 4; ++r) {
                const bool ireal = 16 * ti + kq + 4 * r < np;
#pragma unroll
                for (int tj = 0; tj <= ti; ++tj) {
                    const int t = ti * (ti + 1) / 2 + tj;
                    double bv = kp[fidx[t][r]];
                    asm volatile("" : "+v"(bv));
                    const double padv = (fdiag[t][r] && !ireal) ? 1.0 : 0.0;
// ... 147 lines not shown
```

### ingvio_amd/csrc/kernels_factored.hip

```cpp
#include <algorithm>
#include <stdlib.h>
#include <string.h>
#include "launch_factored.h"

#include "gate_kernel.h"
#include "gate5_kernel.h"
#include "gate5m_kernel.h"

#define GATE_FPW 1
template <int CMAX, bool STEREO>
__global__ __launch_bounds__(GATE_FPW * WAVE) __attribute__((amdgpu_waves_per_eu(2, 4))) void k_feat_gate3(
    CovView cv, FrameView fv, MsckfOpts op, int b0, int nb, int fmax_used, double* __restrict__ gamma_out,
    int* __restrict__ accept_out, double* __restrict__ rec_out)
{
    gate3_body<CMAX, STEREO, GATE_FPW, false>(cv, fv, op, b0, nb, fmax_used, gamma_out, accept_out, rec_out);
}

#ifndef GATE4_WPE
#define GATE4_WPE 2
#endif
#ifndef GATE4_WPE_MAX
#define GATE4_WPE_MAX 6
#endif
template <int CMAX>
__global__ __launch_bounds__(WAVE) __attribute__((amdgpu_waves_per_eu(GATE4_WPE, GATE4_WPE_MAX))) void k_feat_gate4(
    CovView cv, FrameView fv, MsckfOpts op, int b0, int nb, int fmax_used, double* __restrict__ gamma_out, int* __restrict__ accept_out)
{
    gate4_body<CMAX>(cv, fv, op, b0, nb, fmax_used, gamma_out, accept_out);
}

#ifndef GATE5_WPE
#define GATE5_WPE 2
#endif
template <int CMAX>
__global__ __launch_bounds__(WAVE) __attribute__((amdgpu_waves_per_eu(GATE5_WPE, GATE5_WPE))) void k_feat_gate5(
    CovView cv, FrameView fv, MsckfOpts op, int b0, int nb, int fmax_used, double* __restrict__ gamma_out, int* __restrict__ accept_out)
{
    gate5_body<CMAX>(cv, fv, op, b0, nb, fmax_used, gamma_out, accept_out);
}

template <int CMAX>
__global__ __launch_bounds__(WAVE) __attribute__((amdgpu_waves_per_eu(GATE5_WPE, GATE5_WPE))) void k_feat_gate5m(
    CovView cv, FrameView fv, MsckfOpts op, int b0, int nb, int fmax_used, double* __restrict__ gamma_out, int* __restrict__ accept_out)
{
    gate5m_body<CMAX>(cv, fv, op, b0, nb, fmax_used, gamma_out, accept_out);
}

#define GRAM_NB 8
#define GRAM_NT 256
#ifndef GRAM2_ZFORM
#define GRAM2_ZFORM 1
#endif
__device__ __forceinline__ double gram_rsqrt(double x)
{
    double y = __builtin_amdgcn_rsq(x);
    double e = fma(-x * y, y, 1.0);
    y = fma(y * e, fma(e, 0.375, 0.5), y);
    e = fma(-x * y, y, 1.0);
    return fma(y * e, 0.5, y);
}
template <int CMAX>
struct Gram2Cfg {
    static constexpr int NC = 6 * CMAX;
    static constexpr int TI = (NC + 15) / 16;
    static constexpr int TJ = (NC + 1 + 15) / 16;
    static constexpr int LDW = 16 * TJ;
    static constexpr int NTILE = TI * TJ;
    static constexpr int NUP = TI * TJ - TI * (TI - 1) / 2;
    static constexpr int TPW = (NUP + 3) / 4;
    static constexpr int KR = 3 * GRAM_NB;
    static constexpr int SPW = 34;
};
template <int CMAX>
struct Gram2Batch {
    using Cfg = Gram2Cfg<CMAX>;
    double Bm[Cfg::KR][Cfg::LDW];
    double Ym[Cfg::KR][Cfg::LDW];
    double sp[CMAX * CMAX <= 128 ? 2 : 1][GRAM_NB][CMAX][Cfg::SPW];
};
template <int CMAX>
struct Gram2Out {
    using Cfg = Gram2Cfg<CMAX>;
    double A2[Cfg::NC][Cfg::NC + 2];
    double S[CMAX][CMAX][34];
};

template <int CMAX, bool STEREO>
__global__ __launch_bounds__(GRAM_NT, 2) void k_feat_gram2(
    FrameView fv, MsckfOpts op, int b0, const int* __restrict__ accept_in, int* __restrict__ used_out,
    double* __restrict__ Apart, int* __restrict__ chunk_used, int G, int rstride)
{
    using Cfg = Gram2Cfg<CMAX>;
    constexpr int NC = Cfg::NC, TJ = Cfg::TJ, LDW = Cfg::LDW, NTILE = Cfg::NTILE, TPW = Cfg::TPW, KR = Cfg::KR;
    constexpr int NUP = Cfg::NUP, TI = Cfg::TI, RPO = STEREO ? 4 : 2;
    extern __shared__ __attribute__((aligned(16))) char smem_raw[];
    Gram2Batch<CMAX>& sb = *reinterpret_cast<Gram2Batch<CMAX>*>(smem_raw);
    Gram2Out<CMAX>& so = *reinterpret_cast<Gram2Out<CMAX>*>(smem_raw);
    constexpr size_t UNI = sizeof(Gram2Batch<CMAX>) > sizeof(Gram2Out<CMAX>) ? sizeof(Gram2Batch<CMAX>) : sizeof(Gram2Out<CMAX>);
    int* sUse = reinterpret_cast<int*>(smem_raw + ((UNI + 15) / 16) * 16);
    int* sList = sUse + fv.fmax;
    __shared__ int sNu;
    __shared__ double sPose[16][12];
    const int bl = blockIdx.y, b = b0 + bl, g = blockIdx.x, tid = threadIdx.x, lane = tid & 63, wave = __builtin_amdgcn_readfirstlane(tid >> 6);
    const int F = fv.n_feat[b], C = fv.n_clones[b], ncol = 6 * C;
    for (int e = tid; e < 12 * C; e += GRAM_NT) {
        const int c = e / 12, q = e - 12 * c;
        sPose[c][q] = q < 9 ? fv.clone_R[((size_t)b * fv.cmax + c) * 9 + q] : fv.clone_p[((size_t)b * fv.cmax + c) * 3 + q - 9];
    }

    dbg_stamp(32);
    for (int j = tid; j < F; j += GRAM_NT) {
        int use = accept_in[(size_t)b * fv.fmax + j];
        if (use && op.max_accept > 0) {
            int rank = 0;
            for (int q = 0; q < j; ++q) rank += accept_in[(size_t)b * fv.fmax + q];
            if (rank >= op.max_accept) use = 0;
        }
        sUse[j] = use;
        if (g == 0) used_out[(size_t)b * fv.fmax + j] = use;
    }
    for (int e = tid; e < KR * LDW; e += GRAM_NT) { (&sb.Bm[0][0])[e] = 0.0; (&sb.Ym[0][0])[e] = 0.0; }
    __syncthreads();
    if (wave == 0) {
        int cnt = 0;
        for (int base = 0; base < F; base += WAVE) {
            const int j = base + lane;
            const bool u = j < F && sUse[j];
            const unsigned long long m = __ballot(u);
            if (u) sList[cnt + __popcll(m & ((1ULL << lane) - 1ULL))] = j;
            cnt += __popcll(m);
        }
        if (lane == 0) sNu = cnt;
    }
    __syncthreads();
    const int nu = sNu, per = (nu + G - 1) / G;
    const int q0 = g * per, q1 = min(nu, q0 + per);

    dbg_stamp(33);
    int tiA[TPW], tjA[TPW];
#pragma unroll
    for (int u = 0; u < TPW; ++u) {
        int t = wave + 4 * u, ti = 0;
        while (ti < TI - 1 && t >= TJ - ti) { t -= TJ - ti; ++ti; }
        tiA[u] = ti; tjA[u] = ti + t;
    }
    double4_f acc[TPW];
#pragma unroll
    for (int u = 0; u < TPW; ++u) acc[u] = double4_f{ 0.0, 0.0, 0.0, 0.0 };
    constexpr bool OVL = CMAX * CMAX <= 128;
    const int ptid = OVL ? tid - 128 : tid;
    const int pc = ptid >= 0 ? ptid / CMAX : 0, pa = ptid >= 0 ? ptid - pc * CMAX : 0;
    const bool pairlane = ptid >= 0 && ptid < CMAX * CMAX;
    double sS1[9], sNX[9], sS3[9], s4[3], s5[3];
#pragma unroll
    for (int i = 0; i < 9; ++i) { sS1[i] = 0.0; sNX[i] = 0.0; sS3[i] = 0.0; }
#pragma unroll
    for (int i = 0; i < 3; ++i) { s4[i] = 0.0; s5[i] = 0.0; }
#ifndef GRAM2_P3B_UNIFORM
#define GRAM2_P3B_UNIFORM 1
#endif
    constexpr bool P3U = GRAM2_P3B_UNIFORM && CMAX * CMAX <= 128 && 11 * CMAX <= 128;
    double sacc[3 * CMAX];
#pragma unroll
    for (int i = 0; i < 3 * CMAX; ++i) sacc[i] = 0.0;
    const int uc = ptid >= 0 ? ptid / 11 : 0, uj = ptid >= 0 ? ptid - 11 * uc : 0;
    const bool ulane = P3U && ptid >= 0 && ptid < 11 * CMAX;
    const int kq = lane >> 4, l15 = lane & 15;

    double in_uv[4], in_pf[3];
    unsigned long long in_mask = 0ULL;
    int in_anchor = 0;
#ifndef GRAM_SPLIT
#define GRAM_SPLIT 0
#endif
    constexpr bool SPLIT = GRAM_SPLIT && CMAX * CMAX <= 128;
    const int ft = SPLIT ? (tid & 127) : tid;
    auto fetch = [&](int qb) {
        const int f = ft >> 4, c = ft & 15;
        in_mask = 0ULL; in_anchor = 0;
#pragma unroll
        for (int i = 0; i < 4; ++i) in_uv[i] = 0.0;
#pragma unroll
        for (int i = 0; i < 3; ++i) in_pf[i] = 0.0;
        if (ft < GRAM_NB * 16 && qb + f < q1) {
            const size_t oidx = (size_t)b * fv.fmax + sList[qb + f];
            in_mask = fv.obs_mask[oidx]; in_anchor = fv.anchor[oidx];
#pragma unroll
            for (int i = 0; i < 3; ++i) in_pf[i] = fv.pf[oidx * 3 + i];
            if (c < C && ((in_mask >> c) & 1ULL)) {
                const double* z = fv.uv + (oidx * fv.cmax + c) * 4;
                in_uv[0] = z[0]; in_uv[1] = z[1];
                if (STEREO) { in_uv[2] = z[2]; in_uv[3] = z[3]; }
            }
        }
    };
    auto sum16 = [](double v) {
#ifdef GRAM_SHFL_SUM
        v += __shfl_xor(v, 8, 16); v += __shfl_xor(v, 4, 16); v += __shfl_xor(v, 2, 16); v += __shfl_xor(v, 1, 16);
#else
        v += row_ror_f64<8>(v); v += row_ror_f64<4>(v); v += row_ror_f64<2>(v); v += row_ror_f64<1>(v);
#endif
        return v;
    };
    fetch(q0);
    auto do_p2 = [&](int qb, int buf, int nthr, bool rows, bool sparse) {
        const int nbf = min(GRAM_NB, q1 - qb);
        dbg_stamp(34);
        if (rows && nbf < GRAM_NB) {
            for (int e = tid; e < (KR - 3 * nbf) * LDW; e += nthr) { (&sb.Bm[3 * nbf][0])[e] = 0.0; (&sb.Ym[3 * nbf][0])[e] = 0.0; }
        }
        dbg_stamp(35);
        if (ft < nbf * 16) {
            const int f = ft >> 4, c = ft & 15;
            const int a = in_anchor;
            const double px = in_pf[0], py = in_pf[1], pz = in_pf[2];
            bool obs = c < C && ((in_mask >> c) & 1ULL);
            double N[9], h[3];
#pragma unroll
            for (int i = 0; i < 9; ++i) N[i] = 0.0;
#pragma unroll
            for (int i = 0; i < 3; ++i) h[i] = 0.0;
            if (obs) {
                double Gm[RPO][3], rs[RPO];
                obs = feat_obs<STEREO>(sPose[c], sPose[c] + 9, in_uv, px, py, pz, op, Gm, rs);
                if (obs) {
#pragma unroll
                    for (int m = 0; m < 3; ++m) {
#pragma unroll
                        for (int m2 = 0; m2 < 3; ++m2) {
                            double sN = 0.0;
#pragma unroll
                            for (int q = 0; q < RPO; ++q) sN += Gm[q][m] * Gm[q][m2];
                            N[3 * m + m2] = sN;
                        }
                        double hh = 0.0;
#pragma unroll
                        for (int q = 0; q < RPO; ++q) hh += Gm[q][m] * rs[q];
                        h[m] = hh;
                    }
                }
            }
            const double cn = (obs && c != a) ? 1.0 : 0.0, pl = (obs && !(op.selected_variant && c == a)) ? 1.0 : 0.0;
            double Ns[9], hs[3], Nsa[9];
            if (rows) {
                const double n0 = sum16(N[0]), n1 = sum16(N[1]), n2 = sum16(N[2]), n4 = sum16(N[4]), n5 = sum16(N[5]), n8 = sum16(N[8]);
                Ns[0] = n0; Ns[1] = n1; Ns[2] = n2; Ns[3] = n1; Ns[4] = n4; Ns[5] = n5; Ns[6] = n2; Ns[7] = n5; Ns[8] = n8;
#ifdef GRAM_NSA_SUMS
                const double a0 = sum16(cn * N[0]), a1 = sum16(cn * N[1]), a2 = sum16(cn * N[2]), a4 = sum16(cn * N[4]), a5 = sum16(cn * N[5]),
                             a8 = sum16(cn * N[8]);
#else
                const int alane = (lane & 48) | (a & 15);
                const double a0 = n0 - __shfl(N[0], alane, WAVE), a1 = n1 - __shfl(N[1], alane, WAVE), a2 = n2 - __shfl(N[2], alane, WAVE),
                             a4 = n4 - __shfl(N[4], alane, WAVE), a5 = n5 - __shfl(N[5], alane, WAVE), a8 = n8 - __shfl(N[8], alane, WAVE);
#endif
                Nsa[0] = a0; Nsa[1] = a1; Nsa[2] = a2; Nsa[3] = a1; Nsa[4] = a4; Nsa[5] = a5; Nsa[6] = a2; Nsa[7] = a5; Nsa[8] = a8;
#pragma unroll
                for (int i = 0; i < 3; ++i) hs[i] = sum16(h[i]);
            }
            if (c < C) {
                double NX[9];
                mulX(N, px, py, pz, NX);
              if (rows) {
                double Bt[9], Bp[9];
#pragma unroll
                for (int i = 0; i < 9; ++i) { Bt[i] = cn * NX[i]; Bp[i] = -pl * N[i]; }
                if (c == a) {
                    double T[9];
                    mulX(Nsa, px, py, pz, T);
#pragma unroll
                    for (int i = 0; i < 9; ++i) Bt[i] = -T[i];
                }
#if GRAM2_ZFORM
                const double s0 = Ns[0] > 0.0 ? gram_rsqrt(Ns[0]) : 0.0, r0 = s0 * s0;
                const double l10 = Ns[1] * r0, l20 = Ns[2] * r0;
                const double d1 = Ns[4] - l10 * Ns[1], s1 = d1 > 0.0 ? gram_rsqrt(d1) : 0.0, r1 = s1 * s1;
                const double t21 = Ns[5] - l20 * Ns[1], l21 = t21 * r1;
                const double d2 = (Ns[8] - l20 * Ns[2]) - l21 * t21, s2 = d2 > 0.0 ? gram_rsqrt(d2) : 0.0;
#pragma unroll
                for (int q = 0; q < 3; ++q) {
                    {
                        const double y0 = Bt[q], y1 = Bt[3 + q] - l10 * y0, y2 = (Bt[6 + q] - l20 * y0) - l21 * y1;
                        sb.Bm[3 * f + 0][6 * c + q] = s0 * y0; sb.Bm[3 * f + 1][6 * c + q] = s1 * y1; sb.Bm[3 * f + 2][6 * c + q] = s2 * y2;
                    }
                    {
                        const double y0 = Bp[q], y1 = Bp[3 + q] - l10 * y0, y2 = (Bp[6 + q] - l20 * y0) - l21 * y1;
                        sb.Bm[3 * f + 0][6 * c + 3 + q] = s0 * y0; sb.Bm[3 * f + 1][6 * c + 3 + q] = s1 * y1; sb.Bm[3 * f + 2][6 * c + 3 + q] = s2 * y2;
                    }
                }
                if (c == 0) {
                    const double y0 = hs[0], y1 = hs[1] - l10 * y0, y2 = (hs[2] - l20 * y0) - l21 * y1;
                    sb.Bm[3 * f + 0][NC] = s0 * y0; sb.Bm[3 * f + 1][NC] = s1 * y1; sb.Bm[3 * f + 2][NC] = s2 * y2;
                }
#else
                double Nsi[9];
                inv3sym(Ns, Nsi);
                double Yt[9], Yp[9];
                mul33(Nsi, Bt, Yt);
                mul33(Nsi, Bp, Yp);
#pragma unroll
                for (int k = 0; k < 3; ++k)
#pragma unroll
                    for (int q = 0; q < 3; ++q) {
                        sb.Bm[3 * f + k][6 * c + q] = Bt[3 * k + q];
                        sb.Bm[3 * f + k][6 * c + 3 + q] = Bp[3 * k + q];
                        sb.Ym[3 * f + k][6 * c + q] = Yt[3 * k + q];
                        sb.Ym[3 * f + k][6 * c + 3 + q] = Yp[3 * k + q];
                    }
                if (c == 0) {
#pragma unroll
                    for (int k = 0; k < 3; ++k) sb.Bm[3 * f + k][NC] = hs[k];
                }
#endif
              }
              if (sparse) {
                double* sp = sb.sp[buf][f][c < CMAX ? c : 0];
                double S1[9];
                mulXt(NX, px, py, pz, S1);
#pragma unroll
                for (int i = 0; i < 9; ++i) { sp[i] = cn * S1[i]; sp[9 + i] = cn * pl * NX[i]; }
                sp[18] = cn * (pz * h[1] - py * h[2]);
                sp[19] = cn * (px * h[2] - pz * h[0]);
                sp[20] = cn * (py * h[0] - px * h[1]);
#pragma unroll
                for (int i = 0; i < 9; ++i) sp[21 + i] = pl * N[i];
#pragma unroll
                for (int i = 0; i < 3; ++i) sp[30 + i] = pl * h[i];
                sp[33] = (obs || c == 0) ? (double)a : -1.0;
              }
            }
        }
    };
    auto do_p3a = [&](int qb) {
        const int nbf = min(GRAM_NB, q1 - qb);
        const int nst = (3 * nbf + 3) >> 2;
#pragma unroll
        for (int st = 0; st < KR / 4; ++st) {
            if (st < nst) {
#pragma unroll
                for (int u = 0; u < TPW; ++u) {
                    if (wave + 4 * u < NUP) {
                        const int ti = tiA[u], tj = tjA[u];
                        const double af = (GRAM2_ZFORM ? sb.Bm : sb.Ym)[4 * st + kq][16 * ti + l15];
                        const double bf = sb.Bm[4 * st + kq][16 * tj + l15];
                        acc[u] = __builtin_amdgcn_mfma_f64_16x16x4f64(af, bf, acc[u], 0, 0, 0);
                    }
                }
            }
        }
    };
    auto do_p3b = [&](int qb, int buf) {
        const int nbf = min(GRAM_NB, q1 - qb);
        if (P3U) {
            if (ulane) {
#pragma unroll
                for (int f = 0; f < GRAM_NB; ++f) {
                    if (f < nbf) {
                        const double* sp = sb.sp[buf][f][uc];
                        const int af = __builtin_amdgcn_readfirstlane((int)sb.sp[buf][f][0][33]);
                        const double x0 = sp[3 * uj], x1 = sp[3 * uj + 1], x2 = sp[3 * uj + 2];
#pragma unroll
                        for (int a2 = 0; a2 < CMAX; ++a2) {
                            const double m = af == a2 ? 1.0 : 0.0;
                            sacc[3 * a2] = fma(m, x0, sacc[3 * a2]);
                            sacc[3 * a2 + 1] = fma(m, x1, sacc[3 * a2 + 1]);
                            sacc[3 * a2 + 2] = fma(m, x2, sacc[3 * a2 + 2]);
                        }
                    }
                }
            }
        } else if (pairlane) {
#pragma unroll
            for (int f = 0; f < GRAM_NB; ++f) {
                if (f < nbf) {
                    const double* sp = sb.sp[buf][f][pc];
                    const double m = sp[33] == (double)pa ? 1.0 : 0.0;
#pragma unroll
                    for (int i = 0; i < 9; ++i) { sS1[i] = fma(m, sp[i], sS1[i]); sNX[i] = fma(m, sp[9 + i], sNX[i]); sS3[i] = fma(m, sp[21 + i], sS3[i]); }
#pragma unroll
                    for (int i = 0; i < 3; ++i) { s4[i] = fma(m, sp[18 + i], s4[i]); s5[i] = fma(m, sp[30 + i], s5[i]); }
                }
            }
        }
    };
    if (OVL) {
        if (q0 < q1) { if (!SPLIT || wave < 2) do_p2(q0, 0, SPLIT ? 128 : GRAM_NT, true, true); fetch(q0 + GRAM_NB); }
        lds_barrier();
        int it = 0;
        for (int qb = q0; qb < q1; qb += GRAM_NB, ++it) {
            if (it == 3) dbg_stamp(36);
            do_p3a(qb);
            if (it == 3) dbg_stamp(37);
            lds_barrier();
            if (it == 3) dbg_stamp(38);
            if (wave < 2) { if (qb + GRAM_NB < q1) { do_p2(qb + GRAM_NB, (it + 1) & 1, 128, true, !SPLIT); fetch(qb + 2 * GRAM_NB); } }
            else {
                do_p3b(qb, it & 1);
                if (SPLIT && qb + GRAM_NB < q1) { do_p2(qb + GRAM_NB, (it + 1) & 1, 128, false, true); fetch(qb + 2 * GRAM_NB); }
            }
            if (it == 3) dbg_stamp(41);
            lds_barrier();
            if (it == 3) dbg_stamp(42);
        }
    } else {
        for (int qb = q0; qb < q1; qb += GRAM_NB) {
            do_p2(qb, 0, GRAM_NT, true, true);
            lds_barrier();
            fetch(qb + GRAM_NB);
            do_p3a(qb);
            do_p3b(qb, 0);
            lds_barrier();
        }
    }

    dbg_stamp(39);
#pragma unroll
    for (int u = 0; u < TPW; ++u) {
        if (wave + 4 * u < NUP) {
            const int ti = tiA[u], tj = tjA[u];
            const int jc = 16 * tj + l15;
#pragma unroll
            for (int r = 0; r < 4; ++r) {
                const int i = 16 * ti + kq + 4 * r;
                if (i < NC && jc <= NC) so.A2[i][jc] = acc[u][r];
            }
        }
    }
    if (P3U) {
        if (ulane) {
#pragma unroll
            for (int a2 = 0; a2 < CMAX; ++a2)
#pragma unroll
                for (int i = 0; i < 3; ++i) {
                    const int v = 3 * uj + i;
                    so.S[uc][a2][v < 18 ? v : (v < 21 ? v + 9 : (v < 30 ? v - 3 : v))] = sacc[3 * a2 + i];
                }
        }
    } else if (pairlane) {
        double* S = so.S[pc][pa];
#pragma unroll
        for (int i = 0; i < 9; ++i) { S[i] = sS1[i]; S[9 + i] = sNX[i]; S[18 + i] = sS3[i]; }
#pragma unroll
        for (int i = 0; i < 3; ++i) { S[27 + i] = s4[i]; S[30 + i] = s5[i]; }
    }
    __syncthreads();
    double* out = Apart + ((size_t)bl * G + g) * rstride;
    if (pairlane && pc < C && pa < C) {
        const int c = pc, c2 = pa;
        double blk[36];
#pragma unroll
        for (int i = 0; i < 36; ++i) blk[i] = 0.0;
        double bb[6] = { 0.0, 0.0, 0.0, 0.0, 0.0, 0.0 };
        if (c == c2) {
            for (int a = 0; a < C; ++a) {
                const double* S = so.S[c][a];
                const double* Sa = so.S[a][c];
#pragma unroll
                for (int q = 0; q < 3; ++q)
#pragma unroll
                    for (int q2 = 0; q2 < 3; ++q2) {
                        blk[6 * q + q2] += S[3 * q + q2] + Sa[3 * q + q2];
                        blk[6 * q + 3 + q2] -= S[9 + 3 * q2 + q];
                        blk[6 * (3 + q) + q2] -= S[9 + 3 * q + q2];
                        blk[6 * (3 + q) + 3 + q2] += S[18 + 3 * q + q2];
                    }
#pragma unroll
                for (int q = 0; q < 3; ++q) { bb[q] += S[27 + q] - Sa[27 + q]; bb[3 + q] -= S[30 + q]; }
            }
        } else {
            const double* S = so.S[c][c2];
            const double* St = so.S[c2][c];
#pragma unroll
            for (int q = 0; q < 3; ++q)
#pragma unroll
                for (int q2 = 0; q2 < 3; ++q2) {
                    blk[6 * q + q2] = -S[3 * q + q2] - St[3 * q + q2];
                    blk[6 * (3 + q) + q2] = S[9 + 3 * q + q2];
                    blk[6 * q + 3 + q2] = St[9 + 3 * q2 + q];
                }
        }
#pragma unroll
        for (int q = 0; q < 6; ++q) {
#pragma unroll
            for (int q2 = 0; q2 < 6; ++q2)
                {
                const int ri = 6 * c + q, rj = 6 * c2 + q2;
                const double a2 = (ri >> 4) <= (rj >> 4) ? so.A2[ri][rj] : so.A2[rj][ri];
                out[(size_t)ri * (ncol + 1) + rj] = blk[6 * q + q2] - a2;
            }
            if (c == c2) out[(size_t)(6 * c + q) * (ncol + 1) + ncol] = bb[q] - so.A2[6 * c + q][NC];
        }
    }
    if (tid == 0) chunk_used[bl * G + g] = max(0, q1 - q0);
    dbg_stamp(40);
}

#ifdef INGVIO_ALT_KERNELS
#include "gram3_kernel.h"
#endif

#define INFO_NT 512

template <int NC>
__global__ __launch_bounds__(INFO_NT, 2) void k_info_update(
    CovView cv, FrameView fv, int b0, const double* __restrict__ Apart, const int* __restrict__ chunk_used, int G, int rstride,
    const double* __restrict__ noise_all, double* __restrict__ Mall, int mstride, double* __restrict__ Pcall, int ystride,
    double* __restrict__ dx_all, int* __restrict__ m_out, int* __restrict__ nc_out, int* __restrict__ status,
    const int* __restrict__ marg_idx, int* __restrict__ pc_base_out)
{
    constexpr int LA = 2 * NC + 1, MP = (NC + 3) & ~3;
    extern __shared__ __attribute__((aligned(16))) char smem_raw[];
    double* aug = reinterpret_cast<double*>(smem_raw);
    int* sCol = reinterpret_cast<int*>(aug + (size_t)NC * LA);
    __shared__ unsigned long long sBest[2];
    const int bl = blockIdx.x, b = b0 + bl, tid = threadIdx.x;
    const int C = fv.n_clones[b], ncol = 6 * C, n = cv.n[b], ld = cv.ldp;
    double* dx = dx_all + (size_t)b * ld;
    int total = 0;
    for (int g = 0; g < G; ++g) total += chunk_used[bl * G + g];
    if (total == 0) {
        for (int r = tid; r < n; r += INFO_NT) dx[r] = 0.0;
        if (tid == 0) { m_out[bl] = 0; nc_out[bl] = ncol; pc_base_out[bl] = -1; }
        return;
    }
    const double* P = cov_ptr(cv, b);
    const double var = noise_all[bl];
    dbg_stamp(0);
    for (int c = tid; c < NC; c += INFO_NT) { const int cc = c < ncol ? c : 0; sCol[c] = fv.clone_idx[(size_t)b * fv.cmax + cc / 6] + cc % 6; }
    if (tid < 2) sBest[tid] = 0ULL;
    const int tx = tid & 63, ty = tid >> 6;
    for (int i = ty; i < NC; i += INFO_NT / 64) {
#pragma unroll
        for (int jq = 0; jq < (NC + 1 + 63) / 64; ++jq) {
            const int j = tx + 64 * jq;
            if (j > NC) continue;
            const int jj = j == NC ? ncol : j;
            double s = 0.0;
            if (i < ncol && (j < ncol || j == NC)) {
                const size_t e = (size_t)i * (ncol + 1) + jj;
                for (int g0 = 0; g0 < G; g0 += 4) {
                    double t[4];
#pragma unroll
                    for (int u = 0; u < 4; ++u) {
                        const int g = g0 + u;
                        t[u] = (g < G && chunk_used[bl * G + g]) ? Apart[((size_t)bl * G + g) * rstride + e] : 0.0;
                    }
                    s += (t[0] + t[1]) + (t[2] + t[3]);
                }
            }
            aug[i * LA + NC + j] = s;
        }
    }
    __syncthreads();
    dbg_stamp(1);
    const bool fused = marg_idx && marg_idx[bl] >= 0;
    const int contig = __syncthreads_and(tid >= ncol || sCol[tid < NC ? tid : 0] == sCol[0] + tid);
    const bool zero_copy = fused && contig && sCol[0] + ((NC + 3) & ~3) <= ld;
    {
        constexpr int KG = INFO_NT / NC;
        const int j = tid % NC, g = tid / NC;
        if (g < KG) {
            constexpr int NH = (NC + 1) / 2;
            const int gj = sCol[j];
#pragma unroll 1
            for (int h = 0; h < 2; ++h) {
                const int k0 = h * NH;
                double pc[NH];
#pragma unroll
                for (int k = 0; k < NH; ++k) pc[k] = (k0 + k < NC) ? P[gj + (size_t)sCol[k0 + k < NC ? k0 + k : 0] * ld] : 0.0;
                for (int i = g; i < NC; i += KG) {
                    double s = h == 0 ? ((i == j) ? var : 0.0) : aug[i * LA + j];
                    const double* arow = aug + i * LA + NC + k0;
#pragma unroll
                    for (int k = 0; k < NH; ++k) s += (k0 + k < NC ? arow[k] : 0.0) * pc[k];
                    aug[i * LA + j] = s;
                }
            }
        }
    }
    __syncthreads();
    dbg_stamp(2);
    constexpr int TXN = (LA + 1) / 2, TYN = INFO_NT / TXN, RPT = (NC + TYN - 1) / TYN;
    double* rowbuf = aug;
    double* colbuf = aug + LA + 1;
    double* sPivVal = colbuf + NC;
    int* sInv = reinterpret_cast<int*>(sPivVal + NC);
    const int gx = tid % TXN, gy = tid / TXN;
    const bool active = gy < TYN;
    const int j0 = gx, j1 = gx + TXN;
    double v[RPT][2];
#pragma unroll
    for (int q = 0; q < RPT; ++q) {
        const int i = gy + TYN * q;
        v[q][0] = (active && i < NC) ? aug[i * LA + j0] : 0.0;
        v[q][1] = (active && i < NC && j1 < LA) ? aug[i * LA + j1] : 0.0;
        if (active && j0 == 0 && i < NC) {
            const unsigned long long key = ((unsigned long long)__double_as_longlong(fabs(v[q][0])) & ~0xFFULL) | (unsigned long long)(255 - i);
            atomicMax(&sBest[0], key);
        }
    }
    unsigned usedmask = 0u;
    __syncthreads();
    for (int k = 0; k < NC; ++k) {
        const unsigned long long best = sBest[k & 1];
        const int p = 255 - (int)(best & 0xFFULL);
        if (active) {
            if (gy == p % TYN) {
                const int qp = p / TYN;
                double r0 = 0.0, r1 = 0.0;
#pragma unroll
                for (int q = 0; q < RPT; ++q) if (q == qp) { r0 = v[q][0]; r1 = v[q][1]; }
                rowbuf[j0] = r0;
                if (j1 < LA) rowbuf[j1] = r1;
                usedmask |= 1u << qp;
            }
            const int kc = k >= TXN ? 1 : 0;
            if (gx == k - kc * TXN) {
#pragma unroll
                for (int q = 0; q < RPT; ++q) { const int i = gy + TYN * q; if (i < NC) colbuf[i] = kc ? v[q][1] : v[q][0]; }
            }
        }
        if (tid == 0) { sBest[(k + 1) & 1] = 0ULL; sInv[p] = k; if ((best >> 8) == 0ULL) atomicOr(&status[b], 4); }
        __syncthreads();
        if (active) {
            const double piv = rowbuf[k];
            if (tid == 0) sPivVal[k] = piv;
            const double inv = fast_rcp(piv);
            const double r0 = rowbuf[j0], r1 = j1 < LA ? rowbuf[j1] : 0.0;
            const int kn = k + 1, knc = kn >= TXN ? 1 : 0;
            const bool own_next = kn < NC && gx == kn - knc * TXN;
            unsigned long long mykey = 0ULL;
#pragma unroll
            for (int q = 0; q < RPT; ++q) {
                const int i = gy + TYN * q;
                if (i < NC && i != p) {
                    const double f = colbuf[i] * inv;
                    v[q][0] -= f * r0;
                    v[q][1] -= f * r1;
                    if (own_next && !((usedmask >> q) & 1u)) {
                        const double nv = knc ? v[q][1] : v[q][0];
                        const unsigned long long key = ((unsigned long long)__double_as_longlong(fabs(nv)) & ~0xFFULL) | (unsigned long long)(255 - i);
                        mykey = key > mykey ? key : mykey;
                    }
// ... 407 lines not shown
                                                        const int* __restrict__ marg_idx, int msize, const int* __restrict__ pc_base,
                                                        const double* __restrict__ Tall, size_t tstride, int* __restrict__ status)
{
    constexpr int MP = (NC + 3) & ~3, K4 = MP / 4;
    __shared__ double sV[4][16][17];
    const int bl = blockIdx.y, b = b0 + bl;
    const bool upd = m_all[bl] != 0;
    const int midx = marg_idx ? marg_idx[bl] : -1;
    const bool fused = midx >= 0;
    if (!upd && !fused) return;
    const int n = cv.n[b], ld = cv.ldp, no = fused ? n - msize : n, nt = (no + 15) >> 4;
    const int wave = threadIdx.x >> 6, lane = threadIdx.x & 63, l15 = lane & 15, kq = lane >> 4;
    int t = blockIdx.x * 4 + wave;
    if (t >= nt * (nt + 1) / 2) return;
    int ti = (int)((sqrtf(8.0f * (float)t + 1.0f) - 1.0f) * 0.5f);
    while (ti * (ti + 1) / 2 > t) --ti;
    while ((ti + 1) * (ti + 2) / 2 <= t) ++ti;
    const int tj = t - ti * (ti + 1) / 2;
    const double* P = cov_ptr(cv, b);
    double* dst = fused ? cov_alt_ptr(cv, b) : cov_ptr(cv, b);
    const int pcb = upd ? pc_base[bl] : -1;
    const double* Pc = pcb >= 0 ? P + (size_t)pcb * ld : Pcall + (size_t)bl * ystride;
    const double* T = Tall + (size_t)bl * tstride;
    auto src_of = [&](int o) __attribute__((always_inline)) { return (fused && o >= midx) ? o + msize : o; };
    const int col = tj * 16 + l15, row0 = ti * 16 + kq, row2 = ti * 16 + l15, col20 = tj * 16 + kq;
    const bool inner = ti > tj && ti * 16 + 15 < no;
    double pv[4];
    {
        const int sc = src_of(min(col, no - 1));
#pragma unroll
        for (int r = 0; r < 4; ++r) {
            const int row = row0 + 4 * r;
            const double v = APPLY_LOADP(&P[sc + (size_t)src_of(min(row, no - 1)) * ld]);
            pv[r] = v * ((inner || (row < no && col < no && row >= col)) ? 1.0 : 0.0);
        }
    }
    double4_f acc = { 0.0, 0.0, 0.0, 0.0 };
    if (upd) {
        const int ra = src_of(min(ti * 16 + l15, no - 1)), rb = src_of(min(tj * 16 + l15, no - 1));
        double tf[K4], bf[K4];
#pragma unroll
        for (int k4 = 0; k4 < K4; ++k4) tf[k4] = (T + (size_t)(4 * k4) * ld)[ra + kq * ld];
#pragma unroll
        for (int k4 = 0; k4 < K4; ++k4) bf[k4] = (Pc + (size_t)(4 * k4) * ld)[rb + kq * ld];
        __builtin_amdgcn_sched_barrier(0);
#pragma unroll
        for (int k4 = 0; k4 < K4; ++k4) acc = __builtin_amdgcn_mfma_f64_16x16x4f64(tf[k4], bf[k4], acc, 0, 0, 0);
    }
    double v[4], tr[4];
#pragma unroll
    for (int r = 0; r < 4; ++r) { v[r] = pv[r] - acc[r]; sV[wave][kq + 4 * r][l15] = v[r]; }
    __builtin_amdgcn_wave_barrier();
#pragma unroll
    for (int r = 0; r < 4; ++r) tr[r] = sV[wave][l15][kq + 4 * r];
    __builtin_amdgcn_wave_barrier();
    double* d1 = dst + col + (size_t)row0 * ld;
    double* d2 = dst + row2 + (size_t)col20 * ld;
    bool neg_diag = false;
#pragma unroll
    for (int r = 0; r < 4; ++r) {
        const int row = row0 + 4 * r;
        if (inner || (row < no && col < no && row >= col)) APPLY_STORE(d1 + (size_t)(4 * r) * ld, v[r]);
        neg_diag |= row == col && row < no && v[r] < 0.0;
    }
#pragma unroll
    for (int r = 0; r < 4; ++r) {
        const int col2 = col20 + 4 * r;
        if (inner || (row2 < no && col2 < no && row2 > col2)) APPLY_STORE(d2 + (size_t)(4 * r) * ld, tr[r]);
    }
    if (upd && __any(neg_diag) && lane == 0) atomicOr(&status[b], 2);
}

template <int NC>
__global__ __launch_bounds__(256) void k_post_cols(CovView cv, int b0, const double* __restrict__ Mall, int mstride, const double* __restrict__ Pcall,
                                                   int ystride, const int* __restrict__ m_all, const int* __restrict__ pc_base,
                                                   const int* __restrict__ colmap_all, const int* __restrict__ nc_all, int cstride,
                                                   double* __restrict__ Wall, size_t wstride)
{
    constexpr int MP = (NC + 3) & ~3, K4 = MP / 4, JT = (MP + 15) / 16;
    __shared__ __attribute__((aligned(16))) double sZ[16 * JT][17];
    const int bl = blockIdx.y, b = b0 + bl;
    const int nc = nc_all[bl];
    if (nc == 0) return;
    const int n = cv.n[b], ld = cv.ldp, nt = (n + 15) >> 4;
    const int tid = threadIdx.x, wave = tid >> 6, lane = tid & 63, l15 = lane & 15, kq = lane >> 4;
    const int ti = blockIdx.x * 4 + wave;
    const bool upd = m_all[bl] != 0;
    const double* P = cov_ptr(cv, b);
    const int pcb = upd ? pc_base[bl] : -1;
    const double* Pc = pcb >= 0 ? P + (size_t)pcb * ld : Pcall + (size_t)bl * ystride;
    const double* M = Mall + (size_t)bl * mstride;
    const int* cm = colmap_all + (size_t)bl * cstride;
    double* W = Wall + (size_t)bl * wstride;
    const int gcol = cm[min(l15, nc - 1)];
    if (upd) {
        double bfrag[K4];
#pragma unroll
        for (int k4 = 0; k4 < K4; ++k4) bfrag[k4] = Pc[gcol + (size_t)(4 * k4 + kq) * ld];
        for (int t = wave; t < JT; t += 4) {
            double4_f z = { 0.0, 0.0, 0.0, 0.0 };
            const int mr = min(16 * t + l15, MP - 1);
#pragma unroll
            for (int k4 = 0; k4 < K4; ++k4) z = __builtin_amdgcn_mfma_f64_16x16x4f64(M[(size_t)mr * MP + 4 * k4 + kq], bfrag[k4], z, 0, 0, 0);
#pragma unroll
            for (int r = 0; r < 4; ++r) sZ[16 * t + kq + 4 * r][l15] = z[r];
        }
    }
    lds_barrier();
    if (ti >= nt) return;
    double4_f acc = { 0.0, 0.0, 0.0, 0.0 };
    if (upd) {
        const int ra = min(ti * 16 + l15, n - 1);
#pragma unroll
        for (int k4 = 0; k4 < K4; ++k4)
            acc = __builtin_amdgcn_mfma_f64_16x16x4f64((Pc + (size_t)(4 * k4) * ld)[ra + kq * ld], sZ[4 * k4 + kq][l15], acc, 0, 0, 0);
    }
    if (l15 < nc) {
#pragma unroll
        for (int r = 0; r < 4; ++r) {
            const int row = ti * 16 + kq + 4 * r;
            if (row < n) W[row + (size_t)l15 * ld] = P[row + (size_t)gcol * ld] - acc[r];
        }
    }
}

__global__ __launch_bounds__(256) void k_info_dx(CovView cv, int b0, int MP, const double* __restrict__ Mall, int mstride, const double* __restrict__ Pcall,
                                                 int ystride, const int* __restrict__ m_all, const int* __restrict__ pc_base,
                                                 const int* __restrict__ marg_idx, int msize, double* __restrict__ dx_all)
{
    const int bl = blockIdx.y, b = b0 + bl;
    if (m_all[bl] == 0) return;
    const int n = cv.n[b], ld = cv.ldp, r = blockIdx.x * 256 + threadIdx.x;
    if (r >= n) return;
    const double* P = cov_ptr(cv, b);
    const int pcb = pc_base[bl];
    const double* Pc = pcb >= 0 ? P + (size_t)pcb * ld : Pcall + (size_t)bl * ystride;
    const double* tvec = Mall + (size_t)bl * mstride + (size_t)MP * MP;
    const int midx = marg_idx ? marg_idx[bl] : -1;
    double d;
    if (midx >= 0 && r >= midx && r < midx + msize) {
        d = 0.0;
        for (int k = 0; k < MP; ++k) d += Pc[r + (size_t)k * ld] * tvec[k];
    } else {
        double p[4] = { 0.0, 0.0, 0.0, 0.0 };
        for (int k4 = 0; k4 < MP / 4; ++k4)
#pragma unroll
            for (int q = 0; q < 4; ++q) p[q] += Pc[r + (size_t)(4 * k4 + q) * ld] * tvec[4 * k4 + q];
        d = (p[0] + p[1]) + (p[2] + p[3]);
    }
    dx_all[(size_t)b * ld + r] = d;
}

template <int CMAX, bool STEREO>
static void launch_ft(const FactoredLaunch& L, hipStream_t st)
{
    if (L.stage == 0) {
        const int nb8 = (L.nb + 7) / 8 * 8;
#ifdef INGVIO_ALT_KERNELS
        static const bool gate3 = [] { const char* e = getenv("INGVIO_GATE"); return e && e[0] == '3'; }();
#else
        constexpr bool gate3 = false;
#endif
        static const bool gate4 = [] { const char* e = getenv("INGVIO_GATE"); return e && e[0] == '4'; }();
        if constexpr (STEREO && CMAX <= 11) {
            if (!gate3 && !gate4) {
                LAUNCH_GATE(L, (k_feat_gate5<CMAX>), dim3(nb8 * ((L.fmax_used + 3) / 4)), dim3(WAVE), 0, st, L.cv, L.fv, L.op, L.b0, L.nb, L.fmax_used,
                                   L.gamma, L.accept);
                return;
            }
        }
        if constexpr (!STEREO && CMAX == 11) {
            static const bool gate3m = [] { const char* e = getenv("INGVIO_GATE"); return e && e[0] == '3'; }();
            if (!gate3m) {
                LAUNCH_GATE(L, (k_feat_gate5m<CMAX>), dim3(nb8 * ((L.fmax_used + 3) / 4)), dim3(WAVE), 0, st, L.cv, L.fv, L.op, L.b0, L.nb, L.fmax_used,
                                   L.gamma, L.accept);
                return;
            }
        }
        if constexpr (STEREO) {
            if (!gate3) {
                LAUNCH_GATE(L, (k_feat_gate4<CMAX>), dim3(nb8 * L.fmax_used), dim3(WAVE), 0, st, L.cv, L.fv, L.op, L.b0, L.nb, L.fmax_used,
                                   L.gamma, L.accept);
                return;
            }
        }
#ifndef INGVIO_ALT_KERNELS
        if constexpr (!STEREO)
#endif
        LAUNCH_GATE(L, (k_feat_gate3<CMAX, STEREO>), dim3(nb8 * ((L.fmax_used + GATE_FPW - 1) / GATE_FPW)), dim3(GATE_FPW * WAVE), 0, st,
                           L.cv, L.fv, L.op, L.b0, L.nb, L.fmax_used, L.gamma, L.accept, L.rec);
    } else {
#ifdef INGVIO_ALT_KERNELS
        if constexpr (CMAX * CMAX <= 128) {
            static const bool gram3 = [] { const char* e = getenv("INGVIO_GRAM"); return e && e[0] == '3'; }();
            if (gram3) {
                constexpr size_t uni3 = sizeof(Gram3Batch<CMAX>) > sizeof(Gram2Out<CMAX>) ? sizeof(Gram3Batch<CMAX>) : sizeof(Gram2Out<CMAX>);
                const size_t sm3 = ((uni3 + 15) / 16) * 16 + 2 * sizeof(int) * (size_t)L.fv.fmax;
                static size_t attr_sm3 = 0;
                if (sm3 > attr_sm3) {
                    hipFuncSetAttribute((const void*)k_feat_gram3<CMAX, STEREO>, hipFuncAttributeMaxDynamicSharedMemorySize, (int)sm3);
                    attr_sm3 = sm3;
                }
                hipLaunchKernelGGL((k_feat_gram3<CMAX, STEREO>), dim3(L.G, L.nb), dim3(GRAM_NT), sm3, st,
                                   L.fv, L.op, L.b0, L.accept, L.used, L.Apart, L.chunk_used, L.G, L.rstride);
                return;
            }
        }
#endif
        constexpr size_t uni = sizeof(Gram2Batch<CMAX>) > sizeof(Gram2Out<CMAX>) ? sizeof(Gram2Batch<CMAX>) : sizeof(Gram2Out<CMAX>);
        const size_t sm = ((uni + 15) / 16) * 16 + 2 * sizeof(int) * (size_t)L.fv.fmax;
        static size_t attr_sm = 0;
        if (sm > attr_sm) {
            hipFuncSetAttribute((const void*)k_feat_gram2<CMAX, STEREO>, hipFuncAttributeMaxDynamicSharedMemorySize, (int)sm);
            attr_sm = sm;
        }
        hipLaunchKernelGGL((k_feat_gram2<CMAX, STEREO>), dim3(L.G, L.nb), dim3(GRAM_NT), sm, st,
                           L.fv, L.op, L.b0, L.accept, L.used, L.Apart, L.chunk_used, L.G, L.rstride);
    }
}

__global__ __launch_bounds__(256) void k_chunk_sum(const double* __restrict__ Apart, const int* __restrict__ chunk_used, int G, int rstride,
                                                   double* __restrict__ out, int* __restrict__ used_out)
{
    const int bl = blockIdx.y, e = blockIdx.x * 256 + threadIdx.x;
    const int* cu = chunk_used + (size_t)bl * G;
    const double* A = Apart + (size_t)bl * G * rstride;
    unsigned long long mask = 0;
    int total = 0;
    for (int g = 0; g < G; ++g) { mask |= (cu[g] != 0 ? 1ull : 0ull) << g; total += cu[g]; }
    if (e < rstride) {
        double s = 0.0;
#pragma unroll 8
        for (int g = 0; g < G; ++g) {
            const double x = A[(size_t)g * rstride + e];
            s += ((mask >> g) & 1ull) ? x : 0.0;
        }
        out[(size_t)bl * rstride + e] = s;
    }
    if (blockIdx.x == 0 && threadIdx.x == 0) used_out[bl] = total;
}

int factored_rec_size(int cmax)
{
    if (cmax > 16) return cmax <= bigwin_cmax() ? bigwin_rec_size() : 0;
    const int cls = cmax <= 6 ? 6 : (cmax <= 11 ? 11 : (cmax <= 12 ? 12 : 16));
    return rec_size(cls);
}

int launch_factored(const FactoredLaunch& L, hipStream_t st)
{
    if (L.fv.cmax > 16) return launch_bigwin(L, st);
    const int cm_sel = (L.c_used > 0 && L.c_used <= L.fv.cmax) ? L.c_used : L.fv.cmax;
    const int ncm = 6 * cm_sel;
    if (L.stage == 10) {
        const int MP = ncm <= 36 ? 36 : (ncm <= 66 ? 68 : (ncm <= 72 ? 72 : 96));
        hipLaunchKernelGGL(k_info_dx, dim3((L.n_cap + 255) / 256, L.nb), dim3(256), 0, st, L.cv, L.b0, MP, L.T, L.mstride, L.Pc, L.ystride, L.m_out,
                           L.pc_base, L.marg_idx, L.marg_size, L.dx);
        return 0;
    }
    if (L.stage == 4) {
        const int nt = (L.n_cap + 15) / 16;
#define POSTCOLS_DISPATCH(NC)                                                                                           \
        hipLaunchKernelGGL((k_post_cols<NC>), dim3((nt + 3) / 4, L.nb), dim3(256), 0, st, L.cv, L.b0, L.T, L.mstride, L.Pc, L.ystride, L.m_out, \
                           L.pc_base, L.gcolmap, L.gnc, L.gcstride, L.gW, L.gWstride);
        if (ncm <= 36) { POSTCOLS_DISPATCH(36) } else if (ncm <= 66) { POSTCOLS_DISPATCH(66) } else if (ncm <= 72) { POSTCOLS_DISPATCH(72) } else { POSTCOLS_DISPATCH(96) }
#undef POSTCOLS_DISPATCH
        return 0;
    }
    if (L.stage == 3) {
        const int nt = (L.n_cap + 15) / 16, wgpf = ((nt + 1) / 2 + 3) / 4, nb8 = (L.nb + 7) / 8 * 8;
#ifdef INGVIO_ALT_KERNELS
        static const bool tw1 = [] { const char* e = getenv("INGVIO_APPLY_TW"); return !(e && e[0] == '2'); }();
#define APPLY_TW2(NC) else if (!tw1) hipLaunchKernelGGL((k_info_apply<NC, 2>), dim3(nb8 * wgpf), dim3(256), 0, st, L.cv, L.b0, L.nb, wgpf, L.T, L.mstride, L.Pc, \
                           L.ystride, L.m_out, L.dx, L.status, L.marg_idx, L.marg_size, L.pc_base);
#else
#define APPLY_TW2(NC)
#endif
        if (!L.gY && L.Tflat && L.nb <= L.flat_nb) {
            const int JTx = ncm <= 36 ? 3 : (ncm <= 72 ? 5 : 6);
#define FLAT_DISPATCH(NC)                                                                                             \
            hipLaunchKernelGGL((k_apply_T_flat<NC>), dim3((nt * JTx + 3) / 4, L.nb), dim3(256), 0, st, L.cv, L.b0, L.T, L.mstride, L.Pc, L.ystride, \
                               L.m_out, L.marg_idx, L.marg_size, L.pc_base, L.Tflat, L.tfstride, L.dx);                 \
            hipLaunchKernelGGL((k_apply_sym_flat<NC>), dim3((nt * (nt + 1) / 2 + 3) / 4, L.nb), dim3(256), 0, st, L.cv, L.b0, L.Pc, L.ystride, \
                               L.m_out, L.marg_idx, L.marg_size, L.pc_base, L.Tflat, L.tfstride, L.status);
            if (ncm <= 36) { FLAT_DISPATCH(36) } else if (ncm <= 66) { FLAT_DISPATCH(66) } else if (ncm <= 72) { FLAT_DISPATCH(72) } else { FLAT_DISPATCH(96) }
#undef FLAT_DISPATCH
            return 0;
        }
#define APPLY_DISPATCH(NC)                                                                                            \
        if (L.gY) { hipLaunchKernelGGL((k_info_apply<NC, 1, 16>), dim3(nb8 * wgpf), dim3(256), 0, st, L.cv, L.b0, L.nb, wgpf, L.T, L.mstride, L.Pc, \
                           L.ystride, L.m_out, L.dx, L.status, L.marg_idx, L.marg_size, L.pc_base, L.gY, L.gYstride, L.gm, flip); if (flip) *L.did_flip = 1; } \
        APPLY_TW2(NC)                                                                                                 \
        else { hipLaunchKernelGGL((k_info_apply<NC, 1>), dim3(nb8 * wgpf), dim3(256), 0, st, L.cv, L.b0, L.nb, wgpf, L.T, L.mstride, L.Pc, \
                           L.ystride, L.m_out, L.dx, L.status, L.marg_idx, L.marg_size, L.pc_base, (const double*)nullptr, (size_t)0, (const int*)nullptr, flip); if (flip) *L.did_flip = 1; }
        int* const flip = (L.marg_idx && L.did_flip) ? L.flip_cnt : nullptr;
        if (ncm <= 36) { APPLY_DISPATCH(36) } else if (ncm <= 66) { APPLY_DISPATCH(66) } else if (ncm <= 72) { APPLY_DISPATCH(72) } else { APPLY_DISPATCH(96) }
#undef APPLY_DISPATCH
#undef APPLY_TW2
        return 0;
    }
    if (L.stage == 2 && L.G > 1 && L.Asum) {
        hipLaunchKernelGGL(k_chunk_sum, dim3((L.rstride + 255) / 256, L.nb), dim3(256), 0, st, L.Apart, L.chunk_used, L.G, L.rstride, L.Asum, L.used_sum);
        FactoredLaunch L1 = L;
        L1.Apart = L.Asum; L1.chunk_used = L.used_sum; L1.G = 1; L1.Asum = nullptr;
        return launch_factored(L1, st);
    }
    if (L.stage == 2) {
#ifdef INGVIO_ALT_KERNELS
        static const bool use_gj = [] { const char* e = getenv("INGVIO_INFO_SOLVE"); return e && !strcmp(e, "gj"); }();
#else
        constexpr bool use_gj = false;
#endif
        if (!use_gj && launch_info_solve(L, st) == 0) return 0;
#define INFO_DISPATCH(NC)                                                                                                   \
        {                                                                                                                   \
            const size_t sm = sizeof(double) * (size_t)NC * (2 * NC + 1) + sizeof(int) * (size_t)NC + 16;                     \
            hipFuncSetAttribute((const void*)k_info_update<NC>, hipFuncAttributeMaxDynamicSharedMemorySize, (int)sm);         \
            hipLaunchKernelGGL(k_info_update<NC>, dim3(L.nb), dim3(INFO_NT), sm, st, L.cv, L.fv, L.b0, L.Apart, L.chunk_used, \
                               L.G, L.rstride, L.noise, L.T, L.mstride, L.Pc, L.ystride, L.dx, L.m_out, L.nc_out, L.status,  \
                               L.marg_idx, L.pc_base);                                                                      \
        }
        if (ncm <= 36) { INFO_DISPATCH(36) } else if (ncm <= 66) { INFO_DISPATCH(66) } else if (ncm <= 72) { INFO_DISPATCH(72) } else { INFO_DISPATCH(96) }
#undef INFO_DISPATCH
        return 0;
    }
    const int cm = cm_sel;
    const int cls = cm <= 6 ? 6 : (cm <= 11 ? 11 : (cm <= 12 ? 12 : (cm <= 16 ? 16 : -1)));
    if (cls < 0) return -1;
#define DISPATCH(CM)                                                         \
    if (cls == CM) { if (L.stereo) launch_ft<CM, true>(L, st); else launch_ft<CM, false>(L, st); return 0; }
    DISPATCH(6)
    DISPATCH(11)
    DISPATCH(12)
    DISPATCH(16)
#undef DISPATCH
    return -1;
}

int dbg_read_factored(long long* out, int n) { return dbg_read_local(out, n); }
```

### ingvio_amd/csrc/kernels_solve.hip

```cpp
#include <stdlib.h>
#include <string.h>
#include "launch_factored.h"

typedef double double4_f __attribute__((ext_vector_type(4)));

namespace {

template <int NC>
struct SolveCfg {
    static constexpr int NT = (NC + 15) / 16, NP = 16 * NT;
    static constexpr int NR1 = (NC + 1 + 15) / 16, R1ROWS = 16 * NR1;
    static constexpr int NW = 8, RW = 2;
    static constexpr int MROWS = R1ROWS > NP ? R1ROWS : NP, LDM = NP + 1;
    static constexpr int PANROWS = NP + R1ROWS + NP;
    static constexpr int MP = (NC + 3) & ~3;
    static constexpr int LDSS = NC + 6 + 1;
    static constexpr size_t lds_bytes() { return sizeof(double) * (2 * (size_t)MROWS * LDM + 2 * (size_t)PANROWS * 4 + 4 * NP) + sizeof(int) * NP; }
};

struct TileRow { int kind, rt, arow, c0, c1; bool valid; };

template <int NC, int PHASE>
constexpr TileRow row_desc(int i)
{
// ... 232 lines not shown
                    }
                    asm volatile("" : "+v"(x[0]), "+v"(x[1]), "+v"(x[2]), "+v"(x[3]));
#pragma unroll
                    for (int r = 0; r < 4; ++r) {
                        const int row = 16 * D1.rows[W][w].rt + kq + 4 * r;
                        T[w][c][r] = (row < ncol && col < ncol) ? x[r] : (row == col ? 1.0 : 0.0);
                    }
                } else {
#pragma unroll
                    for (int r = 0; r < 4; ++r) T[w][c][r] = (16 * D1.rows[W][w].rt + kq + 4 * r == col) ? 1.0 : 0.0;
                }
            }
        lds_barrier();
        for (int e = W * 64 + lane; e < 2 * MROWS * LDM; e += NTH) X[e] = 0.0;
        lds_barrier();
        auto emit = [&](int w, int row, int col, int k, double x, double xs) {
            if (D1.rows[W][w].kind == 0) X[row * LDM + col] = row > 4 * k + 3 ? xs : (row == col ? 1.0 : 0.0);
            else Y[(row - NP) * LDM + col] = xs;
        };
        dbg_stamp(1);
        ldl_sweep<NC, 1, W>(T, a.pan, lane, emit, a.sD1inv, bad);
    }
    dbg_stamp(2);
#pragma unroll
    for (int w = 0; w < RW; ++w)
#pragma unroll
        for (int c = 0; c < NT; ++c) {
            T[w][c] = double4_f{ 0.0, 0.0, 0.0, 0.0 };
            if (D2.rows[W][w].valid && D2.rows[W][w].kind == 2 && c >= D2.rows[W][w].c0) {
#pragma unroll
                for (int r = 0; r < 4; ++r) T[w][c][r] = Y[(16 * D2.rows[W][w].rt + kq + 4 * r) * LDM + 16 * c + l15];
            }
        }
    lds_barrier();
#pragma unroll
    for (int w = 0; w < RW; ++w) {
        if (D2.rows[W][w].valid && D2.rows[W][w].kind == 1) {
            constexpr int dummy = 0; (void)dummy;
            const int i = D2.rows[W][w].rt;
            if (one_partial) {
#pragma unroll
                for (int kt = 0; kt < NT; ++kt)
#pragma unroll
                    for (int s = 0; s < 4; ++s) af[w][kt][s] = ((okm[w] >> (4 * kt + s)) & 1u) ? af[w][kt][s] : 0.0;
            }
#pragma unroll
            for (int j = 0; j < NT; ++j) {
                double4_f acc = { 0.0, 0.0, 0.0, 0.0 };
#pragma unroll
                for (int kt = j; kt < NT; ++kt)
#pragma unroll
                    for (int s = 0; s < 4; ++s)
                        acc = __builtin_amdgcn_mfma_f64_16x16x4f64(af[w][kt][s], X[(16 * kt + 4 * s + kq) * LDM + 16 * j + l15], acc, 0, 0, 0);
                T[w][j] = acc;
#pragma unroll
                for (int r = 0; r < 4; ++r) Y[(16 * i + kq + 4 * r) * LDM + 16 * j + l15] = acc[r];
            }
        }
    }
    __syncthreads();
    dbg_stamp(3);
#pragma unroll
    for (int w = 0; w < RW; ++w) {
        if (D2.rows[W][w].valid && D2.rows[W][w].kind == 0) {
            constexpr int dummy = 0; (void)dummy;
            const int i = D2.rows[W][w].rt;
            double4_f acc[NT];
#pragma unroll
            for (int j = 0; j < NT; ++j) acc[j] = double4_f{ 0.0, 0.0, 0.0, 0.0 };
#pragma unroll
            for (int kt = 0; kt < NT; ++kt) {
                if (kt >= i) {
#pragma unroll
                    for (int s = 0; s < 4; ++s) {
                        const int kr = 16 * kt + 4 * s + kq;
                        const double afv = X[kr * LDM + 16 * i + l15];
#pragma unroll
                        for (int j = 0; j < NT; ++j)
                            if (j <= i) {
                                const double bfv = (NC < NP && kr >= NC) ? 0.0 : Y[kr * LDM + 16 * j + l15];
                                acc[j] = __builtin_amdgcn_mfma_f64_16x16x4f64(afv, bfv, acc[j], 0, 0, 0);
                            }
                    }
                }
            }
#pragma unroll
            for (int j = 0; j < NT; ++j)
                if (j <= i) {
                    if (j == i) {
#pragma unroll
                        for (int r = 0; r < 4; ++r) {
                            const int rr = kq + 4 * r;
                            if ((l15 >> 2) == r) acc[j][r] += a.var * a.sD1inv[16 * (4 * i + r) + 4 * kq + (l15 & 3)];
                            (void)rr;
                        }
                    }
                    T[w][j] = acc[j];
                }
        }
    }
    __syncthreads();
    dbg_stamp(4);
    for (int e = W * 64 + lane; e < MROWS * LDM; e += NTH) Y[e] = 0.0;
    {
        auto emit = [&](int w, int row, int col, int k, double x, double xs) {
            if (D2.rows[W][w].kind == 1) X[(row - NP) * LDM + col] = xs;
            else if (D2.rows[W][w].kind == 2) Y[(row - NP - R1ROWS) * LDM + col] = x;
        };
        ldl_sweep<NC, 2, W>(T, a.pan, lane, emit, a.sD1inv, bad);
    }
}

template <int NCF, bool RED>
__global__ __launch_bounds__(512) __attribute__((amdgpu_waves_per_eu(4, 4))) void k_info_solve(
    CovView cv, FrameView fv, int b0, const double* __restrict__ Apart, const int* __restrict__ chunk_used, int G, int rstride,
    const double* __restrict__ noise_all, double* __restrict__ Mall, int mstride, double* __restrict__ Pcall, int ystride,
    double* __restrict__ dx_all, int* __restrict__ m_out, int* __restrict__ nc_out, int* __restrict__ status,
    const int* __restrict__ marg_idx, int* __restrict__ pc_base_out)
{
    constexpr int NC = RED ? NCF - 6 : NCF;
    using Cfg = SolveCfg<NC>;
    constexpr int NT = Cfg::NT, NP = Cfg::NP, NR1 = Cfg::NR1, NW = Cfg::NW;
    constexpr int LDM = Cfg::LDM, MROWS = Cfg::MROWS, PANROWS = Cfg::PANROWS, NTH = 64 * NW;
    constexpr int MPF = (NCF + 3) & ~3, NPF = 16 * ((NCF + 15) / 16), CF = NCF / 6;
    extern __shared__ __attribute__((aligned(16))) char smem_raw[];
    double* X = reinterpret_cast<double*>(smem_raw);
    double* Y = X + (size_t)MROWS * LDM;
    double (*pan)[PANROWS][4] = reinterpret_cast<double (*)[PANROWS][4]>(Y + (size_t)MROWS * LDM);
    double* sD1inv = reinterpret_cast<double*>(pan) + 2 * (size_t)PANROWS * 4;
    double* sD2inv = nullptr;
    int* sCol = reinterpret_cast<int*>(sD1inv + 4 * NP);
    __shared__ int sBad, sRefSlot;
    int* sColF = reinterpret_cast<int*>(&pan[1][0][0]);
    int* sRef = sColF + NPF;
    double* sTr = reinterpret_cast<double*>(sRef + NPF + (NPF & 1));
    static_assert(sizeof(int) * (2 * NPF + 2) + sizeof(double) * 256 <= sizeof(double) * PANROWS * 4, "set-up tables exceed a panel buffer");
    dbg_stamp(60);
    const int bl = blockIdx.x, b = b0 + bl, tid = threadIdx.x, wave = __builtin_amdgcn_readfirstlane(tid >> 6), lane = tid & 63;
    const int kq = lane >> 4, l15 = lane & 15;
    const int C = fv.n_clones[b], ncolF = 6 * C, n = cv.n[b], ld = cv.ldp;
    double* dx = dx_all + (size_t)b * ld;
    int total = 0;
    for (int g = 0; g < G; ++g) total += chunk_used[bl * G + g];
    if (total == 0) {
        for (int r = tid; r < n; r += NTH) dx[r] = 0.0;
        if (tid == 0) { m_out[bl] = 0; nc_out[bl] = ncolF; pc_base_out[bl] = -1; }
        return;
    }
    const double* P = cov_ptr(cv, b);
    for (int c = tid; c < NPF; c += NTH) { const int cc = c < ncolF ? c : 0; sColF[c] = fv.clone_idx[(size_t)b * fv.cmax + cc / 6] + cc % 6; }
#ifndef SOLVE_REF_BY_INFO
#define SOLVE_REF_BY_INFO 0
#endif
    if (SOLVE_REF_BY_INFO && RED && tid < 256) {
        const int c = tid >> 4, g0 = tid & 15;
        double tr = 0.0;
        if (c < C) {
            for (int g = g0; g < G; g += 16) {
                const double* Ap = Apart + ((size_t)bl * G + g) * rstride;
                const double u = chunk_used[bl * G + g] ? 1.0 : 0.0;
                const size_t e = (size_t)(6 * c + 3) * (ncolF + 1) + 6 * c + 3;
                tr += u * ((Ap[e] + Ap[e + ncolF + 2]) + Ap[e + 2 * (ncolF + 2)]);
            }
        }
        sTr[tid] = tr;
    }
    if (tid == 0) sBad = 0;
    __syncthreads();
    dbg_stamp(61);
    static_assert((NC + 6) * Cfg::LDSS <= 2 * MROWS * LDM, "the staged window block exceeds the X / Y area");
    {
        constexpr int SPT = (NCF * NCF + NTH - 1) / NTH;
        const int nn = ncolF * ncolF;
        const float inv = 1.0f / (float)ncolF;
        double sv[SPT];
        int so[SPT];
#pragma unroll
        for (int u = 0; u < SPT; ++u) {
            const int e = min(tid + NTH * u, nn - 1);
            const int i = (int)(((float)e + 0.5f) * inv), j = e - i * ncolF;
            sv[u] = P[sColF[j] + (size_t)sColF[i] * ld];
            so[u] = i * Cfg::LDSS + j;
        }
#pragma unroll
        for (int u = 0; u < SPT; ++u) if (tid + NTH * u < nn) X[so[u]] = sv[u];
    }
    if (!SOLVE_REF_BY_INFO && RED && tid == 0) sRefSlot = C - 1;
    if (SOLVE_REF_BY_INFO && RED && tid == 0) {
        int best = 0; double tb = -1.0;
        for (int c = 0; c < C; ++c) {
            double t = 0.0;
            for (int g = 0; g < 16; ++g) t += sTr[16 * c + g];
            if (t > tb) { tb = t; best = c; }
        }
        sRefSlot = best;
    }
    const bool fused = marg_idx && marg_idx[bl] >= 0;
    const int contig = __syncthreads_and(tid >= ncolF || sColF[tid < NPF ? tid : 0] == sColF[0] + tid);
    const bool zero_copy = fused && contig && sColF[0] + MPF <= ld;
    const int ref6 = RED ? 6 * sRefSlot : (1 << 20), ncol = RED ? ncolF - 6 : ncolF;
    for (int c = tid; c < NP; c += NTH) {
        const int cf = c < ncol ? c + (c >= ref6 ? 6 : 0) : 0;
        sCol[c] = sColF[cf];
        if (RED) sRef[c] = sColF[ref6 + cf % 6];
    }
    __syncthreads();
    int bad = 0;
    dbg_stamp(0);
    SolveArgs<NC> sa{ P, sCol, X, Y, pan, sD1inv, sD2inv, Apart, chunk_used, G, rstride, bl, ncol, ld, lane, noise_all[bl], sRef, ncolF, ref6 };
    switch (wave) {
    case 0: solve_wave<NC, 0, RED>(sa, &bad); break;
    case 1: solve_wave<NC, 1, RED>(sa, &bad); break;
    case 2: solve_wave<NC, 2, RED>(sa, &bad); break;
    case 3: solve_wave<NC, 3, RED>(sa, &bad); break;
    case 4: solve_wave<NC, 4, RED>(sa, &bad); break;
    case 5: solve_wave<NC, 5, RED>(sa, &bad); break;
    case 6: solve_wave<NC, 6, RED>(sa, &bad); break;
    default: solve_wave<NC, 7, RED>(sa, &bad); break;
    }
    dbg_stamp(5);
    if (bad) sBad = 1;
    double* Mg = Mall + (size_t)bl * mstride;
    constexpr int NQ = (NT * NR1 + NW - 1) / NW;
    double4_f accs[NQ];
#pragma unroll
    for (int u = 0; u < NQ; ++u) {
        const int q = wave + NW * u;
        double4_f acc = { 0.0, 0.0, 0.0, 0.0 };
        if (q < NT * NR1) {
            const int i = q / NR1, j = q % NR1;
            for (int kt = i; kt < NT; ++kt) {
                double af[4], bf[4];
#pragma unroll
                for (int s = 0; s < 4; ++s) {
                    af[s] = Y[(16 * i + l15) * LDM + 16 * kt + 4 * s + kq];
                    bf[s] = X[(16 * j + l15) * LDM + 16 * kt + 4 * s + kq];
                }
#pragma unroll
                for (int s = 0; s < 4; ++s) acc = __builtin_amdgcn_mfma_f64_16x16x4f64(af[s], bf[s], acc, 0, 0, 0);
            }
            const int col = 16 * j + l15;
            if (RED) {
                const int colF = col + (col >= ref6 ? 6 : 0);
#pragma unroll
                for (int r = 0; r < 4; ++r) {
                    const int row = 16 * i + kq + 4 * r, rowF = row + (row >= ref6 ? 6 : 0);
                    if (row < NC && col < NC) Mg[(size_t)rowF * MPF + colF] = acc[r];
                    if (row < NC && col == NC) Mg[(size_t)MPF * MPF + rowF] = acc[r];
                }
            } else {
#pragma unroll
                for (int r = 0; r < 4; ++r) {
                    const int row = 16 * i + kq + 4 * r;
                    const double v = (row < NC) ? acc[r] : 0.0;
                    if (row < MPF && col < MPF) Mg[(size_t)row * MPF + col] = col < NC ? v : 0.0;
                    if (col == NC && row < MPF) Mg[(size_t)MPF * MPF + row] = v;
                }
            }
        }
        accs[u] = acc;
    }
    if (RED) {
        lds_barrier();
#pragma unroll
        for (int u = 0; u < NQ; ++u) {
            const int q = wave + NW * u;
            if (q < NT * NR1) {
                const int i = q / NR1, j = q % NR1, col = 16 * j + l15;
#pragma unroll
                for (int r = 0; r < 4; ++r) {
                    const int row = 16 * i + kq + 4 * r;
                    if (col < LDM) X[row * LDM + col] = accs[u][r];
                }
            }
        }
        lds_barrier();
        for (int e = tid; e < 2 * 6 * (MPF + 1); e += NTH) {
            const int side = e / (6 * (MPF + 1)), q = e - side * 6 * (MPF + 1), k = q / (MPF + 1), J = q - k * (MPF + 1);
            const bool inref = J >= ref6 && J < ref6 + 6;
            if (J == MPF) {
                if (side == 0) {
                    double s = 0.0;
                    for (int cr = 0; cr < CF - 1; ++cr) s += X[(6 * cr + k) * LDM + NC];
                    Mg[(size_t)MPF * MPF + ref6 + k] = -s;
                }
            } else if (!inref) {
                double s = 0.0;
                if (J < NCF) {
                    const int Jr = J < ref6 ? J : J - 6;
                    for (int cr = 0; cr < CF - 1; ++cr) s += side == 0 ? X[(6 * cr + k) * LDM + Jr] : X[Jr * LDM + 6 * cr + k];
                }
                if (side == 0) Mg[(size_t)(ref6 + k) * MPF + J] = -s; else Mg[(size_t)J * MPF + ref6 + k] = -s;
                if (side == 0 && J < NCF) Y[k * LDM + (J < ref6 ? J : J - 6)] = s;
            }
        }
        if (MPF > NCF) {
            for (int e = tid; e < NCF * (MPF - NCF); e += NTH) {
                const int I = e / (MPF - NCF), J = NCF + e % (MPF - NCF);
                if (I < ref6 || I >= ref6 + 6) { Mg[(size_t)I * MPF + J] = 0.0; Mg[(size_t)J * MPF + I] = 0.0; }
            }
            for (int e = tid; e < (MPF - NCF) * (MPF - NCF); e += NTH)
                Mg[(size_t)(NCF + e / (MPF - NCF)) * MPF + NCF + e % (MPF - NCF)] = 0.0;
            if (tid < MPF - NCF) Mg[(size_t)MPF * MPF + NCF + tid] = 0.0;
        }
        lds_barrier();
        if (tid < 36) {
            const int k = tid / 6, l = tid - 6 * k;
            double s = 0.0;
            for (int c2 = 0; c2 < CF - 1; ++c2) s += Y[k * LDM + 6 * c2 + l];
            Mg[(size_t)(ref6 + k) * MPF + ref6 + l] = s;
        }
    }
    dbg_stamp(6);
    if (sBad && tid == 0) atomicOr(&status[b], 4);
    double* Pc = Pcall + (size_t)bl * ystride;
    if (!zero_copy) {
        const int tx = tid & 63, ty = tid >> 6;
        for (int k = ty; k < MPF; k += NW) {
            const bool real = k < ncolF;
            const int gk = real ? fv.clone_idx[(size_t)b * fv.cmax + k / 6] + k % 6 : 0;
            for (int r = tx; r < n; r += 64) Pc[r + (size_t)k * ld] = real ? P[r + (size_t)gk * ld] : 0.0;
        }
    }
    if (tid == 0) { m_out[bl] = ncolF; nc_out[bl] = ncolF; pc_base_out[bl] = zero_copy ? fv.clone_idx[(size_t)b * fv.cmax] : -1; }
    dbg_stamp(7);
}

}

int launch_info_solve(const FactoredLaunch& L, hipStream_t st)
{
    const int ncm = 6 * ((L.c_used > 0 && L.c_used <= L.fv.cmax) ? L.c_used : L.fv.cmax);
#define SOLVE_DISPATCH(NCF, RED)                                                                                              \
    {                                                                                                                         \
        const size_t sm = SolveCfg<(RED ? NCF - 6 : NCF)>::lds_bytes();                                                       \
        static bool attr_set = false;                                                                                         \
        if (!attr_set) { hipFuncSetAttribute((const void*)k_info_solve<NCF, RED>, hipFuncAttributeMaxDynamicSharedMemorySize, (int)sm); attr_set = true; } \
        hipLaunchKernelGGL((k_info_solve<NCF, RED>), dim3(L.nb), dim3(64 * SolveCfg<NCF>::NW), sm, st, L.cv, L.fv, L.b0, L.Apart, L.chunk_used, L.G, L.rstride, \
                           L.noise, L.T, L.mstride, L.Pc, L.ystride, L.dx, L.m_out, L.nc_out, L.status, L.marg_idx, L.pc_base);       \
        return 0;                                                                                                             \
    }
#ifdef INGVIO_ALT_KERNELS
    static const bool no_gauge = [] { const char* e = getenv("INGVIO_INFO_GAUGE"); return e && !strcmp(e, "off"); }();
#else
    constexpr bool no_gauge = false;
#endif
    const bool red = !L.op.selected_variant && !no_gauge;
    if (ncm <= 36) { if (red) SOLVE_DISPATCH(36, true) else SOLVE_DISPATCH(36, false) }
    if (ncm <= 66) { if (red) SOLVE_DISPATCH(66, true) else SOLVE_DISPATCH(66, false) }
    if (ncm <= 72) { if (red) SOLVE_DISPATCH(72, true) else SOLVE_DISPATCH(72, false) }
#undef SOLVE_DISPATCH
    return 1;
}

int dbg_read_solve(long long* out, int n) { return dbg_read_local(out, n); }
```

### ingvio_amd/csrc/launch_factored.h

```cpp
#pragma once
#include "dev_common.h"

#ifndef INGVIO_APPLY_FLAT_NB
#define INGVIO_APPLY_FLAT_NB 64
#endif
constexpr int APPLY_FLAT_NB = INGVIO_APPLY_FLAT_NB;

struct FactoredLaunch {
    int stage;
    int stereo;
    CovView cv;
    FrameView fv;
    MsckfOpts op;
    int b0, nb, fmax_used;
    double* gamma;
    int* accept;
    int* used;
    double* rec;
    double* Apart;
    double* Asum;
    int* used_sum;
    double* Tflat;
    size_t tfstride;
    int flat_nb;
    int* chunk_used;
    int G, rstride;
    const double* noise;
    double* T;
    int mstride, n_cap;
    double* Pc;
    int ystride;
    double* dx;
    int* m_out;
    int* nc_out;
    int* status;
    const int* marg_idx;
    int marg_size;
    int* pc_base;
    int* flip_cnt;
    int* did_flip;
    double* big_sg;
    double* big_wk;
    int ncol_cap;
    int c_used;
    const int* gcolmap;
    const int* gnc;
    int gcstride;
    double* gW;
    size_t gWstride;
    const double* gY;
    size_t gYstride;
    const int* gm;
    hipEvent_t prof_a, prof_b;
    int* prof_used;
};
#include <hip/hip_ext.h>
#define LAUNCH_GATE(L, kernel, grid, block, shmem, st, ...)                                                             \
    do {                                                                                                                \
        if ((L).prof_a) { hipExtLaunchKernelGGL(kernel, grid, block, shmem, st, (L).prof_a, (L).prof_b, 0, __VA_ARGS__); if ((L).prof_used) *(L).prof_used = 1; } \
        else hipLaunchKernelGGL(kernel, grid, block, shmem, st, __VA_ARGS__);                                           \
    } while (0)

int launch_factored(const FactoredLaunch& L, hipStream_t st);
int launch_info_solve(const FactoredLaunch& L, hipStream_t st);
int dbg_read_solve(long long* out, int n);
int factored_rec_size(int cmax);
int dbg_read_factored(long long* out, int n);

int launch_bigwin(const FactoredLaunch& L, hipStream_t st);
void launch_apply64(const FactoredLaunch& L, hipStream_t st, int mp, double* T, size_t tstride, int ldt);
size_t bigwin_sg_doubles(int G);
size_t bigwin_wk_doubles();
int bigwin_rec_size();
int bigwin_cmax();
int dbg_read_bigwin(long long* out, int n);
```

Before: 1.069 million updates/s.

## Skip newest-clone block in Gram panel and optionally reuse gate-stage normal equations

Measured after the change: 1.075 million updates/s (median of 6 runs). No clear change (+0.6%).

```diff
diff --git a/ingvio_amd/csrc/capi.hip b/ingvio_amd/csrc/capi.hip
--- a/ingvio_amd/csrc/capi.hip
+++ b/ingvio_amd/csrc/capi.hip
@@ -83,6 +83,7 @@
     double* d_Asum = nullptr;
     int* d_used_sum = nullptr;
     struct { std::vector<double> chi2; bool chi2_ok = false; double var = 0.0; int b0 = -1, nb = 0; bool noise_ok = false; } upc;
+    bool info_reduced = false;
     int apply_flipped = 0;
     bool fork_recorded = false;
     unsigned long long* d_tri_mask = nullptr;
@@ -748,7 +749,7 @@
 }
 
 int run_msckf_factored(ingvio_ctx* c, int b0, int nb, const MsckfOpts& op, int stereo, int fmax_used,
-                       const int* marg_idx = nullptr, int marg_size = 0, int phase = 0, bool gnss_fuse = false)
+                       const int* marg_idx = nullptr, int marg_size = 0, int phase = 0, bool gnss_fuse = false, bool frame_step = false)
 {
     FactoredLaunch L;
     memset(&L, 0, sizeof L);
@@ -757,6 +758,8 @@
     L.ncol_cap = 6 * c->d.c_max;
     for (int i = 0; i < nb; ++i) if (c->h_nclones[b0 + i] > L.c_used) L.c_used = c->h_nclones[b0 + i];
     L.gamma = c->d_gamma; L.accept = c->d_accept; L.used = c->d_used; L.rec = c->d_rec;
+    L.gram_red = frame_step && phase == 0 && info_solve_reduced(L);
+    c->info_reduced = L.gram_red != 0;
     L.Apart = c->d_Rpart + (size_t)b0 * c->G * c->rstride; L.chunk_used = c->d_chunk_used + (size_t)b0 * c->G;
     L.G = c->G; L.rstride = c->rstride; L.noise = c->d_noise + b0;
     L.Tflat = c->d_Tflat; L.tfstride = (size_t)c->ldp * 100; L.flat_nb = std::min(c->d.batch, APPLY_FLAT_NB);
@@ -3880,8 +3883,8 @@
         HIPCHK(c, hipMemsetAsync(g.mf, 0, sizeof(int) * (size_t)B, c->st));
         g.own_status = true; g.results = true; g.fused_last = true; g.folded_last = false;
     }
-    int rc = fuse     ? run_msckf_factored(c, 0, B, c->st_op, c->st_stereo, c->st_fmax_used, c->d_idx, 6, 0, gnss_fuse)
-             : lm_oop ? run_msckf_factored(c, 0, B, c->st_op, c->st_stereo, c->st_fmax_used, c->d_zero_idx, 0)
+    int rc = fuse     ? run_msckf_factored(c, 0, B, c->st_op, c->st_stereo, c->st_fmax_used, c->d_idx, 6, 0, gnss_fuse, true)
+             : lm_oop ? run_msckf_factored(c, 0, B, c->st_op, c->st_stereo, c->st_fmax_used, c->d_zero_idx, 0, 0, false, true)
                       : run_msckf(c, 0, B, c->st_op, c->st_stereo, c->st_fmax_used);
     if (rc) return rc;
     if (lm_oop) {
@@ -4092,6 +4095,10 @@
 {
     ENTER(c);
     if (check_range(c, b, 1) || !A_out || !ncol_out) return INGVIO_E_ARG;
+    if (c->method == 1 && c->info_reduced) {
+        c->err = "the last update was an unsplit frame step whose partials leave the newest clone's block out: use ingvio_msckf_update or ingvio_frame_run_phase(.., 1)";
+        return INGVIO_E_UNSUPPORTED;
+    }
     int C = 0;
     if (down_sync(c, &C, c->d_nclones + b, sizeof(int))) return INGVIO_E_HIP;
     const int ncol = 6 * C;
diff --git a/ingvio_amd/csrc/feat_build.h b/ingvio_amd/csrc/feat_build.h
--- a/ingvio_amd/csrc/feat_build.h
+++ b/ingvio_amd/csrc/feat_build.h
@@ -78,6 +78,29 @@
     }
     return !nan;
 }
+
+template <int RPO>
+__device__ __forceinline__ void feat_nh(const double (*Gm)[3], const double* rs, double N[9], double h[3])
+{
+#pragma unroll
+    for (int m = 0; m < 3; ++m) {
+#pragma unroll
+        for (int m2 = m; m2 < 3; ++m2) {
+            double sN = 0.0;
+#pragma unroll
+            for (int q = 0; q < RPO; ++q) sN += Gm[q][m] * Gm[q][m2];
+            N[3 * m + m2] = sN; N[3 * m2 + m] = sN;
+        }
+        double hh = 0.0;
+#pragma unroll
+        for (int q = 0; q < RPO; ++q) hh += Gm[q][m] * rs[q];
+        h[m] = hh;
+    }
+}
+
+#define GREC_PLANES 9
+#define GREC_VWORD (GREC_PLANES * 16)
+#define GREC_STRIDE 160
 
 template <int CMAX, bool STEREO, bool LEAN = false>
 __device__ __forceinline__ int feat_phase1(const FrameView& fv, const MsckfOpts& op, int b, int j, int C,
diff --git a/ingvio_amd/csrc/gate5_kernel.h b/ingvio_amd/csrc/gate5_kernel.h
--- a/ingvio_amd/csrc/gate5_kernel.h
+++ b/ingvio_amd/csrc/gate5_kernel.h
@@ -34,7 +34,7 @@
 
 template <int CMAX>
 __device__ __forceinline__ void gate5_body(CovView cv, FrameView fv, MsckfOpts op, int b0, int nb, int fmax_used, double* __restrict__ gamma_out,
-                                           int* __restrict__ accept_out)
+                                           int* __restrict__ accept_out, double* __restrict__ rec_out)
 {
     using SH = Gate5Shared<CMAX>;
     constexpr int NF = SH::NF, NTL = SH::NTL, NLT = NTL * (NTL + 1) / 2, NPMAX = SH::NPMAX;
@@ -101,21 +101,15 @@
     double u[3] = { 0.0, 0.0, 0.0 }, Ni[9], rr = 0.0;
 #pragma unroll
     for (int i = 0; i < 9; ++i) Ni[i] = 0.0;
+    double* const rp = rec_out ? rec_out + oidx * GREC_STRIDE + sl : nullptr;
+    const bool rwr = rec_out && jok && sl < C;
+    if (rwr && sl == 0) *reinterpret_cast<unsigned*>(rp + GREC_VWORD) = gm;
     if (valid) {
         double N[9], h[3];
-#pragma unroll
-        for (int m = 0; m < 3; ++m) {
-#pragma unroll
-            for (int m2 = m; m2 < 3; ++m2) {
-                double sN = 0.0;
-#pragma unroll
-                for (int q = 0; q < 4; ++q) sN += Gm[q][m] * Gm[q][m2];
-                N[3 * m + m2] = sN; N[3 * m2 + m] = sN;
-            }
-            double hh = 0.0;
-#pragma unroll
-            for (int q = 0; q < 4; ++q) hh += Gm[q][m] * rs[q];
-            h[m] = hh;
+        feat_nh<4>(Gm, rs, N, h);
+        if (rwr) {
+            rp[0] = N[0]; rp[16] = N[1]; rp[32] = N[2]; rp[48] = N[4]; rp[64] = N[5]; rp[80] = N[8];
+            rp[96] = h[0]; rp[112] = h[1]; rp[128] = h[2];
         }
         inv3sym(N, Ni);
 #pragma unroll
@@ -125,6 +119,9 @@
             u[m] = Ni[3 * m] * h[0] + Ni[3 * m + 1] * h[1] + Ni[3 * m + 2] * h[2];
             rr -= h[m] * u[m];
         }
+    } else if (rwr) {
+#pragma unroll
+        for (int i = 0; i < GREC_PLANES; ++i) rp[16 * i] = 0.0;
     }
 #pragma unroll
     for (int off = 8; off > 0; off >>= 1) rr += __shfl_xor(rr, off, WAVE);
diff --git a/ingvio_amd/csrc/kernels_factored.hip b/ingvio_amd/csrc/kernels_factored.hip
--- a/ingvio_amd/csrc/kernels_factored.hip
+++ b/ingvio_amd/csrc/kernels_factored.hip
@@ -34,9 +34,10 @@
 #endif
 template <int CMAX>
 __global__ __launch_bounds__(WAVE) __attribute__((amdgpu_waves_per_eu(GATE5_WPE, GATE5_WPE))) void k_feat_gate5(
-    CovView cv, FrameView fv, MsckfOpts op, int b0, int nb, int fmax_used, double* __restrict__ gamma_out, int* __restrict__ accept_out)
-{
-    gate5_body<CMAX>(cv, fv, op, b0, nb, fmax_used, gamma_out, accept_out);
+    CovView cv, FrameView fv, MsckfOpts op, int b0, int nb, int fmax_used, double* __restrict__ gamma_out, int* __restrict__ accept_out,
+    double* __restrict__ rec_out)
+{
+    gate5_body<CMAX>(cv, fv, op, b0, nb, fmax_used, gamma_out, accept_out, rec_out);
 }
 
 template <int CMAX>
@@ -59,11 +60,12 @@
     e = fma(-x * y, y, 1.0);
     return fma(y * e, 0.5, y);
 }
-template <int CMAX>
+template <int CMAX, bool RED = false>
 struct Gram2Cfg {
     static constexpr int NC = 6 * CMAX;
-    static constexpr int TI = (NC + 15) / 16;
-    static constexpr int TJ = (NC + 1 + 15) / 16;
+    static constexpr int NCP = RED ? NC - 6 : NC;
+    static constexpr int TI = (NCP + 15) / 16;
+    static constexpr int TJ = (NCP + 1 + 15) / 16;
     static constexpr int LDW = 16 * TJ;
     static constexpr int NTILE = TI * TJ;
     static constexpr int NUP = TI * TJ - TI * (TI - 1) / 2;
@@ -71,39 +73,42 @@
     static constexpr int KR = 3 * GRAM_NB;
     static constexpr int SPW = 34;
 };
-template <int CMAX>
+template <int CMAX, bool RED = false>
 struct Gram2Batch {
-    using Cfg = Gram2Cfg<CMAX>;
+    using Cfg = Gram2Cfg<CMAX, RED>;
     double Bm[Cfg::KR][Cfg::LDW];
+#if !GRAM2_ZFORM
     double Ym[Cfg::KR][Cfg::LDW];
+#endif
     double sp[CMAX * CMAX <= 128 ? 2 : 1][GRAM_NB][CMAX][Cfg::SPW];
 };
-template <int CMAX>
+template <int CMAX, bool RED = false>
 struct Gram2Out {
-    using Cfg = Gram2Cfg<CMAX>;
-    double A2[Cfg::NC][Cfg::NC + 2];
+    using Cfg = Gram2Cfg<CMAX, RED>;
+    double A2[Cfg::NCP][Cfg::NCP + 2];
     double S[CMAX][CMAX][34];
 };
 
-template <int CMAX, bool STEREO>
+template <int CMAX, bool STEREO, bool REC = false, bool RED = false>
 __global__ __launch_bounds__(GRAM_NT, 2) void k_feat_gram2(
     FrameView fv, MsckfOpts op, int b0, const int* __restrict__ accept_in, int* __restrict__ used_out,
-    double* __restrict__ Apart, int* __restrict__ chunk_used, int G, int rstride)
-{
-    using Cfg = Gram2Cfg<CMAX>;
-    constexpr int NC = Cfg::NC, TJ = Cfg::TJ, LDW = Cfg::LDW, NTILE = Cfg::NTILE, TPW = Cfg::TPW, KR = Cfg::KR;
+    double* __restrict__ Apart, int* __restrict__ chunk_used, int G, int rstride, const double* __restrict__ rec)
+{
+    using Cfg = Gram2Cfg<CMAX, RED>;
+    constexpr int NC = Cfg::NC, NCP = Cfg::NCP, TJ = Cfg::TJ, LDW = Cfg::LDW, TPW = Cfg::TPW, KR = Cfg::KR;
     constexpr int NUP = Cfg::NUP, TI = Cfg::TI, RPO = STEREO ? 4 : 2;
+    static_assert(!REC || STEREO, "the record is written by the stereo gate");
     extern __shared__ __attribute__((aligned(16))) char smem_raw[];
-    Gram2Batch<CMAX>& sb = *reinterpret_cast<Gram2Batch<CMAX>*>(smem_raw);
-    Gram2Out<CMAX>& so = *reinterpret_cast<Gram2Out<CMAX>*>(smem_raw);
-    constexpr size_t UNI = sizeof(Gram2Batch<CMAX>) > sizeof(Gram2Out<CMAX>) ? sizeof(Gram2Batch<CMAX>) : sizeof(Gram2Out<CMAX>);
+    Gram2Batch<CMAX, RED>& sb = *reinterpret_cast<Gram2Batch<CMAX, RED>*>(smem_raw);
+    Gram2Out<CMAX, RED>& so = *reinterpret_cast<Gram2Out<CMAX, RED>*>(smem_raw);
+    constexpr size_t UNI = sizeof(Gram2Batch<CMAX, RED>) > sizeof(Gram2Out<CMAX, RED>) ? sizeof(Gram2Batch<CMAX, RED>) : sizeof(Gram2Out<CMAX, RED>);
     int* sUse = reinterpret_cast<int*>(smem_raw + ((UNI + 15) / 16) * 16);
     int* sList = sUse + fv.fmax;
     __shared__ int sNu;
     __shared__ double sPose[16][12];
     const int bl = blockIdx.y, b = b0 + bl, g = blockIdx.x, tid = threadIdx.x, lane = tid & 63, wave = __builtin_amdgcn_readfirstlane(tid >> 6);
     const int F = fv.n_feat[b], C = fv.n_clones[b], ncol = 6 * C;
-    for (int e = tid; e < 12 * C; e += GRAM_NT) {
+    for (int e = tid; e < (REC ? 0 : 12 * C); e += GRAM_NT) {
         const int c = e / 12, q = e - 12 * c;
         sPose[c][q] = q < 9 ? fv.clone_R[((size_t)b * fv.cmax + c) * 9 + q] : fv.clone_p[((size_t)b * fv.cmax + c) * 3 + q - 9];
     }
@@ -119,7 +124,12 @@
         sUse[j] = use;
         if (g == 0) used_out[(size_t)b * fv.fmax + j] = use;
     }
-    for (int e = tid; e < KR * LDW; e += GRAM_NT) { (&sb.Bm[0][0])[e] = 0.0; (&sb.Ym[0][0])[e] = 0.0; }
+    for (int e = tid; e < KR * LDW; e += GRAM_NT) {
+        (&sb.Bm[0][0])[e] = 0.0;
+#if !GRAM2_ZFORM
+        (&sb.Ym[0][0])[e] = 0.0;
+#endif
+    }
     __syncthreads();
     if (wave == 0) {
         int cnt = 0;
@@ -167,8 +177,9 @@
     const bool ulane = P3U && ptid >= 0 && ptid < 11 * CMAX;
     const int kq = lane >> 4, l15 = lane & 15;
 
-    double in_uv[4], in_pf[3];
+    double in_uv[REC ? GREC_PLANES : 4], in_pf[3];
     unsigned long long in_mask = 0ULL;
+    unsigned in_vw = 0u;
     int in_anchor = 0;
 #ifndef GRAM_SPLIT
 #define GRAM_SPLIT 0
@@ -178,8 +189,9 @@
     auto fetch = [&](int qb) {
         const int f = ft >> 4, c = ft & 15;
         in_mask = 0ULL; in_anchor = 0;
-#pragma unroll
-        for (int i = 0; i < 4; ++i) in_uv[i] = 0.0;
+        in_vw = 0u;
+#pragma unroll
+        for (int i = 0; i < (REC ? GREC_PLANES : 4); ++i) in_uv[i] = 0.0;
 #pragma unroll
         for (int i = 0; i < 3; ++i) in_pf[i] = 0.0;
         if (ft < GRAM_NB * 16 && qb + f < q1) {
@@ -187,7 +199,14 @@
             in_mask = fv.obs_mask[oidx]; in_anchor = fv.anchor[oidx];
 #pragma unroll
             for (int i = 0; i < 3; ++i) in_pf[i] = fv.pf[oidx * 3 + i];
-            if (c < C && ((in_mask >> c) & 1ULL)) {
+            if constexpr (REC) {
+                const double* rp = rec + oidx * GREC_STRIDE;
+                in_vw = *reinterpret_cast<const unsigned*>(rp + GREC_VWORD);
+                if (c < C && ((in_mask >> c) & 1ULL)) {
+#pragma unroll
+                    for (int i = 0; i < GREC_PLANES; ++i) in_uv[i] = rp[16 * i + c];
+                }
+            } else if (c < C && ((in_mask >> c) & 1ULL)) {
                 const double* z = fv.uv + (oidx * fv.cmax + c) * 4;
                 in_uv[0] = z[0]; in_uv[1] = z[1];
                 if (STEREO) { in_uv[2] = z[2]; in_uv[3] = z[3]; }
@@ -207,7 +226,12 @@
         const int nbf = min(GRAM_NB, q1 - qb);
         dbg_stamp(34);
         if (rows && nbf < GRAM_NB) {
-            for (int e = tid; e < (KR - 3 * nbf) * LDW; e += nthr) { (&sb.Bm[3 * nbf][0])[e] = 0.0; (&sb.Ym[3 * nbf][0])[e] = 0.0; }
+            for (int e = tid; e < (KR - 3 * nbf) * LDW; e += nthr) {
+                (&sb.Bm[3 * nbf][0])[e] = 0.0;
+#if !GRAM2_ZFORM
+                (&sb.Ym[3 * nbf][0])[e] = 0.0;
+#endif
+            }
         }
         dbg_stamp(35);
         if (ft < nbf * 16) {
@@ -220,25 +244,17 @@
             for (int i = 0; i < 9; ++i) N[i] = 0.0;
 #pragma unroll
             for (int i = 0; i < 3; ++i) h[i] = 0.0;
-            if (obs) {
+            if constexpr (REC) {
+                obs = obs && ((in_vw >> c) & 1u);
+                if (obs) {
+                    N[0] = in_uv[0]; N[1] = in_uv[1]; N[2] = in_uv[2]; N[3] = in_uv[1]; N[4] = in_uv[3]; N[5] = in_uv[4];
+                    N[6] = in_uv[2]; N[7] = in_uv[4]; N[8] = in_uv[5];
+                    h[0] = in_uv[6]; h[1] = in_uv[7]; h[2] = in_uv[8];
+                }
+            } else if (obs) {
                 double Gm[RPO][3], rs[RPO];
                 obs = feat_obs<STEREO>(sPose[c], sPose[c] + 9, in_uv, px, py, pz, op, Gm, rs);
-                if (obs) {
-#pragma unroll
-                    for (int m = 0; m < 3; ++m) {
-#pragma unroll
-                        for (int m2 = 0; m2 < 3; ++m2) {
-                            double sN = 0.0;
-#pragma unroll
-                            for (int q = 0; q < RPO; ++q) sN += Gm[q][m] * Gm[q][m2];
-                            N[3 * m + m2] = sN;
-                        }
-                        double hh = 0.0;
-#pragma unroll
-                        for (int q = 0; q < RPO; ++q) hh += Gm[q][m] * rs[q];
-                        h[m] = hh;
-                    }
-                }
+                if (obs) feat_nh<RPO>(Gm, rs, N, h);
             }
             const double cn = (obs && c != a) ? 1.0 : 0.0, pl = (obs && !(op.selected_variant && c == a)) ? 1.0 : 0.0;
             double Ns[9], hs[3], Nsa[9];
@@ -276,20 +292,21 @@
                 const double d1 = Ns[4] - l10 * Ns[1], s1 = d1 > 0.0 ? gram_rsqrt(d1) : 0.0, r1 = s1 * s1;
                 const double t21 = Ns[5] - l20 * Ns[1], l21 = t21 * r1;
                 const double d2 = (Ns[8] - l20 * Ns[2]) - l21 * t21, s2 = d2 > 0.0 ? gram_rsqrt(d2) : 0.0;
+                const bool zcols = !(RED && c == CMAX - 1);
 #pragma unroll
                 for (int q = 0; q < 3; ++q) {
-                    {
+                    if (zcols) {
                         const double y0 = Bt[q], y1 = Bt[3 + q] - l10 * y0, y2 = (Bt[6 + q] - l20 * y0) - l21 * y1;
                         sb.Bm[3 * f + 0][6 * c + q] = s0 * y0; sb.Bm[3 * f + 1][6 * c + q] = s1 * y1; sb.Bm[3 * f + 2][6 * c + q] = s2 * y2;
                     }
-                    {
+                    if (zcols) {
                         const double y0 = Bp[q], y1 = Bp[3 + q] - l10 * y0, y2 = (Bp[6 + q] - l20 * y0) - l21 * y1;
                         sb.Bm[3 * f + 0][6 * c + 3 + q] = s0 * y0; sb.Bm[3 * f + 1][6 * c + 3 + q] = s1 * y1; sb.Bm[3 * f + 2][6 * c + 3 + q] = s2 * y2;
                     }
                 }
                 if (c == 0) {
                     const double y0 = hs[0], y1 = hs[1] - l10 * y0, y2 = (hs[2] - l20 * y0) - l21 * y1;
-                    sb.Bm[3 * f + 0][NC] = s0 * y0; sb.Bm[3 * f + 1][NC] = s1 * y1; sb.Bm[3 * f + 2][NC] = s2 * y2;
+                    sb.Bm[3 * f + 0][NCP] = s0 * y0; sb.Bm[3 * f + 1][NCP] = s1 * y1; sb.Bm[3 * f + 2][NCP] = s2 * y2;
                 }
 #else
                 double Nsi[9];
@@ -301,6 +318,7 @@
                 for (int k = 0; k < 3; ++k)
 #pragma unroll
                     for (int q = 0; q < 3; ++q) {
+                        if (RED && c == CMAX - 1) continue;
                         sb.Bm[3 * f + k][6 * c + q] = Bt[3 * k + q];
                         sb.Bm[3 * f + k][6 * c + 3 + q] = Bp[3 * k + q];
                         sb.Ym[3 * f + k][6 * c + q] = Yt[3 * k + q];
@@ -308,7 +326,7 @@
                     }
                 if (c == 0) {
 #pragma unroll
-                    for (int k = 0; k < 3; ++k) sb.Bm[3 * f + k][NC] = hs[k];
+                    for (int k = 0; k < 3; ++k) sb.Bm[3 * f + k][NCP] = hs[k];
                 }
 #endif
               }
@@ -340,7 +358,11 @@
                 for (int u = 0; u < TPW; ++u) {
                     if (wave + 4 * u < NUP) {
                         const int ti = tiA[u], tj = tjA[u];
-                        const double af = (GRAM2_ZFORM ? sb.Bm : sb.Ym)[4 * st + kq][16 * ti + l15];
+#if GRAM2_ZFORM
+                        const double af = sb.Bm[4 * st + kq][16 * ti + l15];
+#else
+                        const double af = sb.Ym[4 * st + kq][16 * ti + l15];
+#endif
                         const double bf = sb.Bm[4 * st + kq][16 * tj + l15];
                         acc[u] = __builtin_amdgcn_mfma_f64_16x16x4f64(af, bf, acc[u], 0, 0, 0);
                     }
@@ -421,7 +443,7 @@
 #pragma unroll
             for (int r = 0; r < 4; ++r) {
                 const int i = 16 * ti + kq + 4 * r;
-                if (i < NC && jc <= NC) so.A2[i][jc] = acc[u][r];
+                if (i < NCP && jc <= NCP) so.A2[i][jc] = acc[u][r];
             }
         }
     }
@@ -484,10 +506,11 @@
             for (int q2 = 0; q2 < 6; ++q2)
                 {
                 const int ri = 6 * c + q, rj = 6 * c2 + q2;
+                if (RED && (c == CMAX - 1 || c2 == CMAX - 1)) { out[(size_t)ri * (ncol + 1) + rj] = blk[6 * q + q2]; continue; }
                 const double a2 = (ri >> 4) <= (rj >> 4) ? so.A2[ri][rj] : so.A2[rj][ri];
                 out[(size_t)ri * (ncol + 1) + rj] = blk[6 * q + q2] - a2;
             }
-            if (c == c2) out[(size_t)(6 * c + q) * (ncol + 1) + ncol] = bb[q] - so.A2[6 * c + q][NC];
+            if (c == c2) out[(size_t)(6 * c + q) * (ncol + 1) + ncol] = (RED && c == CMAX - 1) ? bb[q] : bb[q] - so.A2[6 * c + q][NCP];
         }
     }
     if (tid == 0) chunk_used[bl * G + g] = max(0, q1 - q0);
@@ -1201,6 +1224,31 @@
 }
 
 template <int CMAX, bool STEREO>
+static bool gram_rec_on(const FactoredLaunch& L)
+{
+    if constexpr (STEREO && CMAX <= 11) {
+        static const bool on = [] { const char* e = getenv("INGVIO_GRAM_REC"); return e && !strcmp(e, "on"); }();
+        static const bool other_gate = [] { const char* e = getenv("INGVIO_GATE"); return e && (e[0] == '3' || e[0] == '4'); }();
+        return on && !other_gate && L.rec != nullptr;
+    }
+    return false;
+}
+
+template <int CMAX, bool STEREO, bool REC, bool RED>
+static void launch_gram2(const FactoredLaunch& L, hipStream_t st)
+{
+    constexpr size_t uni = sizeof(Gram2Batch<CMAX, RED>) > sizeof(Gram2Out<CMAX, RED>) ? sizeof(Gram2Batch<CMAX, RED>) : sizeof(Gram2Out<CMAX, RED>);
+    const size_t sm = ((uni + 15) / 16) * 16 + 2 * sizeof(int) * (size_t)L.fv.fmax;
+    static size_t attr_sm = 0;
+    if (sm > attr_sm) {
+        hipFuncSetAttribute((const void*)k_feat_gram2<CMAX, STEREO, REC, RED>, hipFuncAttributeMaxDynamicSharedMemorySize, (int)sm);
+        attr_sm = sm;
+    }
+    hipLaunchKernelGGL((k_feat_gram2<CMAX, STEREO, REC, RED>), dim3(L.G, L.nb), dim3(GRAM_NT), sm, st,
+                       L.fv, L.op, L.b0, L.accept, L.used, L.Apart, L.chunk_used, L.G, L.rstride, (const double*)L.rec);
+}
+
+template <int CMAX, bool STEREO>
 static void launch_ft(const FactoredLaunch& L, hipStream_t st)
 {
     if (L.stage == 0) {
@@ -1213,8 +1261,13 @@
         static const bool gate4 = [] { const char* e = getenv("INGVIO_GATE"); return e && e[0] == '4'; }();
         if constexpr (STEREO && CMAX <= 11) {
             if (!gate3 && !gate4) {
+#ifdef GRAM_ABL_REC
+                double* const recw = nullptr;
+#else
+                double* const recw = gram_rec_on<CMAX, STEREO>(L) ? L.rec : nullptr;
+#endif
                 LAUNCH_GATE(L, (k_feat_gate5<CMAX>), dim3(nb8 * ((L.fmax_used + 3) / 4)), dim3(WAVE), 0, st, L.cv, L.fv, L.op, L.b0, L.nb, L.fmax_used,
-                                   L.gamma, L.accept);
+                                   L.gamma, L.accept, recw);
                 return;
             }
         }
@@ -1256,15 +1309,21 @@
             }
         }
 #endif
-        constexpr size_t uni = sizeof(Gram2Batch<CMAX>) > sizeof(Gram2Out<CMAX>) ? sizeof(Gram2Batch<CMAX>) : sizeof(Gram2Out<CMAX>);
-        const size_t sm = ((uni + 15) / 16) * 16 + 2 * sizeof(int) * (size_t)L.fv.fmax;
-        static size_t attr_sm = 0;
-        if (sm > attr_sm) {
-            hipFuncSetAttribute((const void*)k_feat_gram2<CMAX, STEREO>, hipFuncAttributeMaxDynamicSharedMemorySize, (int)sm);
-            attr_sm = sm;
-        }
-        hipLaunchKernelGGL((k_feat_gram2<CMAX, STEREO>), dim3(L.G, L.nb), dim3(GRAM_NT), sm, st,
-                           L.fv, L.op, L.b0, L.accept, L.used, L.Apart, L.chunk_used, L.G, L.rstride);
+        bool red = false;
+        if constexpr (CMAX <= 12) {
+            static const bool red_off = [] { const char* e = getenv("INGVIO_GRAM_RED"); return e && !strcmp(e, "off"); }();
+            red = L.gram_red && !red_off;
+        }
+        if constexpr (STEREO && CMAX <= 11) {
+            if (gram_rec_on<CMAX, STEREO>(L)) {
+                if (red) launch_gram2<CMAX, STEREO, true, true>(L, st); else launch_gram2<CMAX, STEREO, true, false>(L, st);
+                return;
+            }
+        }
+        if constexpr (CMAX <= 12) {
+            if (red) { launch_gram2<CMAX, STEREO, false, true>(L, st); return; }
+        }
+        launch_gram2<CMAX, STEREO, false, false>(L, st);
     }
 }
 
@@ -1293,7 +1352,7 @@
 {
     if (cmax > 16) return cmax <= bigwin_cmax() ? bigwin_rec_size() : 0;
     const int cls = cmax <= 6 ? 6 : (cmax <= 11 ? 11 : (cmax <= 12 ? 12 : 16));
-    return rec_size(cls);
+    return std::max(rec_size(cls), GREC_STRIDE);
 }
 
 int launch_factored(const FactoredLaunch& L, hipStream_t st)
diff --git a/ingvio_amd/csrc/kernels_solve.hip b/ingvio_amd/csrc/kernels_solve.hip
--- a/ingvio_amd/csrc/kernels_solve.hip
+++ b/ingvio_amd/csrc/kernels_solve.hip
@@ -408,6 +408,7 @@
 #ifndef SOLVE_REF_BY_INFO
 #define SOLVE_REF_BY_INFO 0
 #endif
+    static_assert(!SOLVE_REF_BY_INFO, "the Gram kernel's reduced panel relies on the newest-clone reference: build it with the full panel before choosing the reference by information");
     if (SOLVE_REF_BY_INFO && RED && tid < 256) {
         const int c = tid >> 4, g0 = tid & 15;
         double tr = 0.0;
@@ -584,6 +585,20 @@
 
 }
 
+bool info_solve_reduced(const FactoredLaunch& L)
+{
+    const int ncm = 6 * ((L.c_used > 0 && L.c_used <= L.fv.cmax) ? L.c_used : L.fv.cmax);
+#ifdef INGVIO_ALT_KERNELS
+    static const bool no_gauge = [] {
+        const char* e = getenv("INGVIO_INFO_GAUGE"); const char* s = getenv("INGVIO_INFO_SOLVE");
+        return (e && !strcmp(e, "off")) || (s && !strcmp(s, "gj"));
+    }();
+#else
+    constexpr bool no_gauge = false;
+#endif
+    return ncm <= 72 && !L.op.selected_variant && !no_gauge;
+}
+
 int launch_info_solve(const FactoredLaunch& L, hipStream_t st)
 {
     const int ncm = 6 * ((L.c_used > 0 && L.c_used <= L.fv.cmax) ? L.c_used : L.fv.cmax);
@@ -596,12 +611,7 @@
                            L.noise, L.T, L.mstride, L.Pc, L.ystride, L.dx, L.m_out, L.nc_out, L.status, L.marg_idx, L.pc_base);       \
         return 0;                                                                                                             \
     }
-#ifdef INGVIO_ALT_KERNELS
-    static const bool no_gauge = [] { const char* e = getenv("INGVIO_INFO_GAUGE"); return e && !strcmp(e, "off"); }();
-#else
-    constexpr bool no_gauge = false;
-#endif
-    const bool red = !L.op.selected_variant && !no_gauge;
+    const bool red = info_solve_reduced(L);
     if (ncm <= 36) { if (red) SOLVE_DISPATCH(36, true) else SOLVE_DISPATCH(36, false) }
     if (ncm <= 66) { if (red) SOLVE_DISPATCH(66, true) else SOLVE_DISPATCH(66, false) }
     if (ncm <= 72) { if (red) SOLVE_DISPATCH(72, true) else SOLVE_DISPATCH(72, false) }
diff --git a/ingvio_amd/csrc/launch_factored.h b/ingvio_amd/csrc/launch_factored.h
--- a/ingvio_amd/csrc/launch_factored.h
+++ b/ingvio_amd/csrc/launch_factored.h
@@ -17,6 +17,7 @@
     int* accept;
     int* used;
     double* rec;
+    int gram_red;
     double* Apart;
     double* Asum;
     int* used_sum;
@@ -63,6 +64,7 @@
 
 int launch_factored(const FactoredLaunch& L, hipStream_t st);
 int launch_info_solve(const FactoredLaunch& L, hipStream_t st);
+bool info_solve_reduced(const FactoredLaunch& L);
 int dbg_read_solve(long long* out, int n);
 int factored_rec_size(int cmax);
 int dbg_read_factored(long long* out, int n);
```
